# gcorso/disco-diffdock

Hardware: AMD Instinct MI355X
Metric: complexes/sec, 20-step 40-sample inference (higher is better)
Workload: dtype f32

## Files before the change

disco_diffdock_amd/csrc/ddk_capi.hip:

```cpp
#include <math.h>
#include <algorithm>
#include <cmath>
#include <string.h>

#include "model.h"
#include "k_conv_common.h"

using namespace ddk;

namespace ddk {


int fail(ddk_ctx* ctx, int code, const std::string& msg) {
  if (ctx) ctx->err = msg;
  return code;
}

int hip_fail(ddk_ctx* ctx, hipError_t e, const char* what) {
  return fail(ctx, DDK_ERR_HIP, std::string(what) + ": " + hipGetErrorString(e));
}

hipError_t ctx_malloc(ddk_ctx* ctx, void** p, size_t bytes) {
  *p = nullptr;
  if (ctx->alloc_limit > 0 && ctx->dev_bytes + (int64_t)bytes > ctx->alloc_limit) { ctx->alloc_refusals++; return hipErrorOutOfMemory; }
// ... 240 lines not shown
        }
        if (n_x > 0 && (int)xs.size() == n_x) {
          std::vector<TileDesc> keep_t; std::vector<TRow> keep_r, x_r; std::vector<int> x_off;
          for (int t = t_first; t < (int)tiles.size(); ++t) {
            if (std::find(xs.begin(), xs.end(), t) != xs.end()) { x_r.push_back(trows[t]); x_off.push_back(tiles[t].w0 >> 16); }
            else { keep_t.push_back(tiles[t]); keep_r.push_back(trows[t]); }
          }
          for (int u = 0; u < 3 * n_x; ++u) {
            keep_r[u].has_x = true; keep_r[u].xpair = u % 3;
            for (int j = 0; j < 4; ++j) keep_r[u].xr[j] = x_r[u / 3].r[j];
            keep_t[u].w0 |= 0x80 | ((u % 3) << 8) | ((x_off[u / 3] / 4) << 10);
          }
          tiles.resize(t_first); trows.resize(t_first);
          tiles.insert(tiles.end(), keep_t.begin(), keep_t.end());
          trows.insert(trows.end(), keep_r.begin(), keep_r.end());
        }
      }
      tiles.back().w0 |= (vec ? FL_V : FL_S) << 2;
    }
  }
  if (mode == 3 && !ctx->cfg.deterministic) {
    L.n_cols = 0;
    for (int t = 0; t < (int)tiles.size(); ++t) {
      const bool prev_flushes = t > 0 && ((tiles[t - 1].w0 >> 2) & 3) != FL_NONE;
      if (t == 0 || prev_flushes || t - L.col_start[L.n_cols - 1] == 2) {
        if (L.n_cols >= 16) return fail(ctx, DDK_ERR_INVALID, "too many output columns");
        if (t > 0 && !prev_flushes) tiles[t - 1].w0 |= FL_V << 2;
        L.col_start[L.n_cols++] = t;
      }
    }
  }
  L.n_tiles = (int)tiles.size();
  L.col_start[L.n_cols] = L.n_tiles;
  L.h_tiles = tiles;

  rowmap.assign((size_t)L.n_tiles * 32, -1);
  rowscale.assign((size_t)L.n_tiles * 32, 0.f);
  for (int t = 0; t < L.n_tiles; ++t) {
    const TRow& tr = trows[t];
    for (int rq = 0; rq < 4; ++rq)
      for (int hh = 0; hh < 2; ++hh)
        for (int j = 0; j < 4; ++j) {
          if (tr.has_x && rq == 3) {
            rowmap[(size_t)t * 32 + 8 * rq + 4 * hh + j] = tr.xr[j].wbase + 8 * tr.col + 2 * tr.xpair + hh;
            rowscale[(size_t)t * 32 + 8 * rq + 4 * hh + j] = tr.xr[j].scale;
            continue;
          }
          const int k = 8 * tr.col + 2 * rq + hh;
          if (!tr.ok[j] || k >= L.n_out[tr.blk[j]]) continue;
          rowmap[(size_t)t * 32 + 8 * rq + 4 * hh + j] = tr.r[j].wbase + k;
          rowscale[(size_t)t * 32 + 8 * rq + 4 * hh + j] = tr.r[j].scale;
        }
  }
  std::vector<int> cnt(L.W, 0);
  for (int r : rowmap) if (r >= 0) cnt[r]++;
  for (int r = 0; r < L.W; ++r) if (cnt[r] != 1) return fail(ctx, DDK_ERR_INVALID, "internal: weight row map is not a bijection");
  return DDK_OK;
}

static int fold_batch_norm(ddk_ctx* ctx, const std::string& pre, const int* out, float* mean, float* scale, float* bias) {
  for (int i = 0; i < XW; ++i) { mean[i] = 0.f; scale[i] = 1.f; bias[i] = 0.f; }
  const int nf = out[0] + out[1] + out[2] + out[3];
  const HostTensor* bw = find_w(ctx, pre + ".weight", {nf});
  const HostTensor* bb = find_w(ctx, pre + ".bias", {out[0]});
  const HostTensor* bm = find_w(ctx, pre + ".running_mean", {out[0]});
  const HostTensor* bv = find_w(ctx, pre + ".running_var", {nf});
  if (!bw || !bb || !bm || !bv) return DDK_ERR_INVALID;
  int ch = 0, f = 0;
  const int dims[4] = {1, 3, 3, 1};
  for (int b = 0; b < 4; ++b)
    for (int m = 0; m < out[b]; ++m, ++f) {
      const float sc = powf(bv->data[f] + 1e-5f, -0.5f) * bw->data[f];
      for (int d = 0; d < dims[b]; ++d, ++ch) {
        scale[ch] = sc;
        if (b == 0) { mean[ch] = bm->data[m]; bias[ch] = bb->data[m]; }
      }
    }
  return DDK_OK;
}

static int pack_x3(ddk_ctx* ctx, ConvLayerDev& L, int NG, const std::vector<float>& w1all, const std::vector<float>& w2all,
                   const std::vector<float>& b2all) {
  const size_t w1sz = 3 * 9 * 64 * 4, w2sz = (size_t)L.n_tiles * 9 * 64 * 4, b2sz = (size_t)L.n_tiles * 32;
  bool exact = true;
  auto split = [&exact](float v, uint16_t& hi, uint16_t& mid, uint16_t& lo) {
    const _Float16 h = (_Float16)v;
    const float r1 = v - (float)h;
    const _Float16 m = (_Float16)r1;
    const _Float16 l = (_Float16)(r1 - (float)m);
    memcpy(&hi, &h, 2); memcpy(&mid, &m, 2); memcpy(&lo, &l, 2);
    const double back = (double)(float)h + (double)(float)m + (double)(float)l;
    if (std::fabs(v) >= 0.5f ? back != (double)v : std::fabs(back - (double)v) > 0x1p-25) exact = false;
  };
  auto range_scale = [](const float* v, size_t n, const float* v2, size_t n2) {
    float m = 0.f;
    for (size_t i = 0; i < n; ++i) m = std::max(m, std::fabs(v[i]));
    for (size_t i = 0; i < n2; ++i) m = std::max(m, std::fabs(v2[i]));
    int e = 0;
    std::frexp(std::max(m, 0x1p-40f), &e);
    return std::ldexp(1.0f, 15 - e);
  };
  std::vector<uint8_t> w2x((size_t)(NG * L.n_tiles + 4) * W2X_TILE_BYTES, 0), w1x((size_t)NG * 3 * W1X_TILE_BYTES, 0);
  auto frags = [&](const float* src, float sc, uint8_t* dst) {
    for (int r = 0; r < 36; ++r)
      for (int lane = 0; lane < 64; ++lane) {
        const float v = src[((size_t)(r / 4) * 64 + lane) * 4 + (r & 3)] * sc;
        const int s_ = r / 8, i = r % 8;
        const size_t off = s_ < 4 ? (size_t)s_ * 1024 + lane * 16 + 2 * i : (size_t)4096 + lane * 8 + 2 * i;
        uint16_t h, m, l;
        split(v, h, m, l);
        memcpy(dst + off, &h, 2); memcpy(dst + W2X_LIMB_BYTES + off, &m, 2); memcpy(dst + 2 * W2X_LIMB_BYTES + off, &l, 2);
      }
  };
  for (int g = 0; g < NG; ++g) {
    const float* w2 = w2all.data() + g * w2sz;
    const float* w1 = w1all.data() + g * w1sz;
    const float* b2 = b2all.data() + g * b2sz;
    const float sc1 = range_scale(w1, w1sz, nullptr, 0), sc2 = range_scale(w2, w2sz, nullptr, 0);
    L.w1s[g] = sc1; L.w2s[g] = sc2;
    for (int t = 0; t < L.n_tiles; ++t) {
      uint8_t* rec = w2x.data() + ((size_t)g * L.n_tiles + t) * W2X_TILE_BYTES;
      frags(w2 + (size_t)t * 2304, sc2, rec);
      memcpy(rec + W2X_BIAS_OFF, b2 + (size_t)t * 32, 128);
      const int32_t dq[2] = {x_tile_word(L.h_tiles[t].w0), L.h_tiles[t].chan0};
      if (dq[0] < 0) return fail(ctx, DDK_ERR_INVALID, "internal: a vector tile of the conv layout does not sit on a T1O / T1E row quad");
      memcpy(rec + W2X_DESC_OFF, dq, 8);
    }
    for (int T = 0; T < 3; ++T) frags(w1 + (size_t)T * 2304, sc1, w1x.data() + ((size_t)g * 3 + T) * W1X_TILE_BYTES);
  }
  if (!exact) return fail(ctx, DDK_ERR_INVALID, "internal: the three-limb fp16 split of a conv weight is not exact");
  L.h_w2x = w2x; L.h_w1x = w1x;
  L.epi_ok = conv_epilogue_shapes_ok(L.h_tiles);
  L.limbs = ctx->cfg.conv_kernel == 3 ? 3 : 2;
  if (ctx->host_only) return DDK_OK;
  L.w2x = (uint8_t*)dev_alloc(ctx, w2x.size());
  L.w1x = (uint8_t*)dev_alloc(ctx, w1x.size());
  if (!L.w2x || !L.w1x) return fail(ctx, DDK_ERR_NOMEM, "device allocation failed while packing conv weights (three-limb f16)");
  if (hipMemcpy(L.w2x, w2x.data(), w2x.size(), hipMemcpyHostToDevice) != hipSuccess ||
      hipMemcpy(L.w1x, w1x.data(), w1x.size(), hipMemcpyHostToDevice) != hipSuccess)
    return fail(ctx, DDK_ERR_HIP, "three-limb weight upload failed");
  return DDK_OK;
}

static int build_conv_layer(ddk_ctx* ctx, int mode, int l, ConvLayerDev& L) {
  const ddk_config& c = ctx->cfg;
  const int ns = c.ns;
  std::vector<int> rowmap;
  std::vector<float> rowscale;
  std::vector<TileDesc> tiles;
  int rc = build_layout(ctx, mode, l, L, rowmap, rowscale, tiles);
  if (rc) return rc;
  const int NG = mode == 0 ? 4 : 9;
  L.n_groups = NG;
  const int ne = 3 * ns;
  auto fc_name = [&](int g) { return mode == 0 ? "conv_layers." + std::to_string(l) + ".fc." + std::to_string(g) : "conv_layers." + std::to_string(9 * l + g) + ".fc"; };
  const std::string lin2 = mode == 0 ? ".4" : ".3";
  if (ctx->weights.find(fc_name(0) + ".0.weight") == ctx->weights.end()) {
    L.has_weights = false;
    return DDK_OK;
  }
  L.has_weights = true;
  const size_t w1sz = 3 * 9 * 64 * 4, b1sz = 3 * 2 * 16, w2sz = (size_t)L.n_tiles * 9 * 64 * 4, b2sz = (size_t)L.n_tiles * 32;
  std::vector<float> w1all(NG * w1sz, 0.f), b1all(NG * b1sz, 0.f), w2all(NG * w2sz, 0.f), b2all(NG * b2sz, 0.f);
  for (int g = 0; g < NG; ++g) {
    const std::string f = fc_name(g);
    const HostTensor* W1 = find_w(ctx, f + ".0.weight", {ne, ne});
    const HostTensor* B1 = find_w(ctx, f + ".0.bias", {ne});
    const HostTensor* W2 = find_w(ctx, f + lin2 + ".weight", {L.W, ne});
    const HostTensor* B2 = find_w(ctx, f + lin2 + ".bias", {L.W});
    if (!W1 || !B1 || !W2 || !B2) return DDK_ERR_INVALID;
    float* w1 = w1all.data() + g * w1sz;
    float* b1 = b1all.data() + g * b1sz;
    float* w2 = w2all.data() + g * w2sz;
    float* b2 = b2all.data() + g * b2sz;
    for (int T = 0; T < 3; ++T) {
      for (int s = 0; s < 36; ++s)
        for (int lane = 0; lane < 64; ++lane) {
          const int hidden = 32 * T + (lane & 31), hh = lane >> 5;
          w1[(((size_t)T * 9 + s / 4) * 64 + lane) * 4 + (s & 3)] = hidden < ne ? W1->data[(size_t)hidden * ne + kin_of(s, hh)] : 0.f;
        }
      for (int hh = 0; hh < 2; ++hh)
        for (int r = 0; r < 16; ++r) {
          const int hidden = 32 * T + d_row(r, hh);
          b1[(T * 2 + hh) * 16 + r] = hidden < ne ? B1->data[hidden] : 0.f;
        }
    }
    for (int t = 0; t < L.n_tiles; ++t) {
      for (int s = 0; s < 36; ++s)
        for (int lane = 0; lane < 64; ++lane) {
          const int row = rowmap[(size_t)t * 32 + (lane & 31)], hh = lane >> 5;
          w2[(((size_t)t * 9 + s / 4) * 64 + lane) * 4 + (s & 3)] =
              row >= 0 ? W2->data[(size_t)row * ne + hid_of(s, hh)] * rowscale[(size_t)t * 32 + (lane & 31)] : 0.f;
        }
      for (int hh = 0; hh < 2; ++hh)
        for (int r = 0; r < 16; ++r) {
          const int row = rowmap[(size_t)t * 32 + d_row(r, hh)];
          b2[((size_t)t * 2 + hh) * 16 + r] = row >= 0 ? B2->data[row] * rowscale[(size_t)t * 32 + d_row(r, hh)] : 0.f;
        }
    }
  }
  if (mode == 0) {
    L.h_wn.assign((size_t)2 * 4 * NE * NS, 0.f);
    L.h_bnp.assign((size_t)2 * 4 * NE, 0.f);
    const int recv_g[2][2] = {{0, 1}, {2, 3}}, send_g[2][2] = {{0, 3}, {1, 2}};
    for (int type = 0; type < 2; ++type)
      for (int slot = 0; slot < 4; ++slot) {
        const int g = slot < 2 ? recv_g[type][slot] : send_g[type][slot - 2];
        const HostTensor* W1 = find_w(ctx, fc_name(g) + ".0.weight", {ne, ne});
        const HostTensor* B1 = find_w(ctx, fc_name(g) + ".0.bias", {ne});
        if (!W1 || !B1) return DDK_ERR_INVALID;
        const int col0 = slot < 2 ? NS : 2 * NS;
        for (int o = 0; o < ne; ++o) {
          const size_t row = ((size_t)(type * 4 + slot) * NE + pre_pos(o));
          for (int k = 0; k < NS; ++k) L.h_wn[row * NS + k] = W1->data[(size_t)o * ne + col0 + k];
          L.h_bnp[row] = slot < 2 ? B1->data[o] : 0.f;
        }
      }
  }
  const int n_bn = mode == 0 ? 1 : NG;
  L.h_bn_mean.assign((size_t)n_bn * XW, 0.f);
  L.h_bn_scale.assign((size_t)n_bn * XW, 1.f);
  L.h_bn_bias.assign((size_t)n_bn * XW, 0.f);
  if (c.batch_norm)
// ... 428 lines not shown
```

disco_diffdock_amd/csrc/ddk_internal.h:

```cpp
#pragma once
#include <hip/hip_runtime.h>
#include <stdint.h>

#include <map>
#include <string>
#include <vector>

#include "../../include/ddk.h"
#include "../../include/ddk_debug.h"

namespace ddk {

constexpr int NS = 24;
constexpr int NV = 6;
constexpr int XW = 2 * NS + 6 * NV;
constexpr int NE = 3 * NS;
constexpr int OFF_P = NS;
constexpr int OFF_Q = NS + 3 * NV;
constexpr int OFF_C = NS + 6 * NV;

constexpr int F_A = 0;
constexpr int F_C = NS;
constexpr int F_T1O = 2 * NS;
constexpr int F_T1E = F_T1O + 6 * NV;
constexpr int F_PQ = F_T1E + 6 * NV;
constexpr int F_STRIDE = F_PQ + 12;
static_assert(F_STRIDE == 132 && NV == 6, "F row layout");

constexpr int F_T2O = F_STRIDE;
constexpr int F_T2E = F_T2O + 24;
constexpr int F_STRIDE2 = F_T2E + 24;
static_assert(F_STRIDE2 == 180, "F row layout (l<=2)");

constexpr int CONV_WAVES = 8;
constexpr int CONV_BLOCK_EDGES = 32 * CONV_WAVES;
constexpr int W2_TILE_FLOATS = 9 * 64 * 4 + 32 + 4;
constexpr int CONV_LDS_FLOATS = CONV_WAVES * 32 * F_STRIDE + 2 * W2_TILE_FLOATS + 16;
constexpr size_t CONV_LDS_BYTES = (size_t)CONV_LDS_FLOATS * 4;
static_assert(CONV_LDS_BYTES <= 160 * 1024, "LDS budget");
template <int MODE> struct ConvTraits;
template <> struct ConvTraits<0> { static constexpr int WAVES = CONV_WAVES, FS = F_STRIDE; };
template <> struct ConvTraits<1> { static constexpr int WAVES = 6, FS = F_STRIDE2; };
template <int MODE> constexpr size_t conv_lds_bytes() { return (size_t)(ConvTraits<MODE>::WAVES * 32 * ConvTraits<MODE>::FS + 2 * W2_TILE_FLOATS + 16) * 4; }
static_assert(conv_lds_bytes<1>() <= 160 * 1024, "LDS budget (l<=2)");
constexpr int CONV_MAX_GROUPS = 9;
constexpr int W2X_LIMB_BYTES = 4 * 1024 + 512;
constexpr int W2X_BIAS_OFF = 3 * W2X_LIMB_BYTES;
constexpr int W2X_DESC_OFF = W2X_BIAS_OFF + 128;
constexpr int W2X_TILE_BYTES = W2X_DESC_OFF + 16;
constexpr int W1X_TILE_BYTES = 3 * W2X_LIMB_BYTES;
constexpr int CONV_TRACE_TILES = 1024;
constexpr int FX_A = 0, FX_C = NS, FX_R = 2 * NS, FX_PQ = FX_R + 6 * NV, FX_STRIDE = FX_PQ + 12 + 4;
static_assert(FX_STRIDE == 100 && FX_A == F_A && FX_C == F_C, "F row layout (three-limb f16)");
constexpr int W2X_STAGES = 4;
constexpr size_t CONV_X_LDS_BYTES = (size_t)CONV_WAVES * 32 * FX_STRIDE * 4 + W2X_STAGES * W2X_TILE_BYTES + 16;
static_assert(CONV_X_LDS_BYTES <= 160 * 1024 && W2X_TILE_BYTES % 16 == 0, "LDS budget (three-limb f16)");

enum TileKind : int {
  T_RA = 0,
  T_RT = 1,
  T_TV = 2,
  T_RTS = 3
};
enum FlushMode : int { FL_NONE = 0, FL_S = 1 , FL_V = 2  };

struct TileDesc {
  int32_t w0;
  int32_t chan0;
  int32_t pad0, pad1;
};
static inline TileDesc make_tile(int kind, int f_off, int flush, int nrq, int chan0) {
  TileDesc t;
  t.w0 = kind | (flush << 2) | (nrq << 4) | (f_off << 16);
  t.chan0 = chan0; t.pad0 = 0; t.pad1 = 0;
  return t;
}

constexpr int32_t X_TILE_L2 = 1 << 24;
static inline int32_t x_tile_word(int32_t w0) {
  const int kind = w0 & 3, f_off = w0 >> 16;
  int nf = f_off;
  if (kind == T_RT || kind == T_RTS) nf = FX_PQ + (f_off - F_PQ);
  else if (kind == T_TV && f_off >= F_T2O) {
    const bool odd = f_off < F_T2E;
    const int rel = f_off - (odd ? F_T2O : F_T2E), q = rel / 12;
    if (f_off >= F_STRIDE2 || rel % 12 || q > 1 || (w0 & 0xc000)) return -1;
    nf = FX_R + 12 * (odd ? q : q + 1);
    return (w0 & 0xffff) | (nf << 16) | X_TILE_L2;
  } else if (kind == T_TV) {
    const bool odd = f_off < F_T1E;
    const int rel = f_off - (odd ? F_T1O : F_T1E), q = rel / 12;
    if (f_off < F_T1O || f_off >= F_PQ || rel % 12 || (w0 & 0xc000)) return -1;
    nf = FX_R + 12 * q;
    for (int half = 0; half < 2; ++half) {
      const bool first = 4 * q + 2 * half < NV;
      if (first != odd) w0 |= 0x4000 << half;
    }
  }
  return (w0 & 0xffff) | (nf << 16);
}

struct ConvLayerDev {
  int n_tiles = 0;
  bool has_weights = false;
  int W = 0;
  int din = 0, dout = 0;
  float* w1p[4] = {};
  float* b1p[4] = {};
  float* w2r[4] = {};
  uint8_t* w1x = nullptr;
  uint8_t* w2x = nullptr;
  float w1s[CONV_MAX_GROUPS] = {1, 1, 1, 1, 1, 1, 1, 1, 1}, w2s[CONV_MAX_GROUPS] = {1, 1, 1, 1, 1, 1, 1, 1, 1};
  int limbs = 2;
  bool epi_ok = false;
  int n_cols = 0;
  int col_start[17] = {};
  float* wn = nullptr;
  float* bnp = nullptr;
  std::vector<float> h_wn, h_bnp;
  float* bn_mean = nullptr;
  float* bn_scale = nullptr;
  float* bn_bias = nullptr;
  std::vector<std::vector<float>> h_w1p, h_b1p, h_w2p, h_b2p;
  std::vector<float> h_bn_mean, h_bn_scale, h_bn_bias;
  int n_groups = 4;
  std::vector<TileDesc> h_tiles;
  std::vector<uint8_t> h_w1x, h_w2x;
  int n_in[4] = {}, n_out[4] = {}, blk_off[4] = {};
  int in_mul[4] = {}, out_mul[4] = {};
};

constexpr int PRE_W = 4 * NE;
static inline int pre_pos(int o) {
  const int r32 = o < 64 ? o % 32 : o - 64, hh = (r32 >> 2) & 1;
  return o < 64 ? hh * 36 + (o / 32) * 16 + (r32 & 3) + 4 * (r32 >> 3) : hh * 36 + 32 + (r32 & 3);
}

struct HostTensor {
  std::vector<int64_t> shape;
// ... 119 lines not shown
```

disco_diffdock_amd/csrc/k_conv_x.hip:

```cpp
#include <stdlib.h>

#include "k_conv_common.h"

#ifdef X3_TWO_LIMBS
#define conv_x3_kernel conv_x2_kernel
#define launch_conv_fused_x launch_conv_fused_x2
#define conv_prepare_device_x conv_prepare_device_x2
#include "k_conv_x_epi2_gen.inc"
#define X3_SUM(r) D0[r]
#define X3_TAIL3(a_lh, a_hm) (void)(a_lh); D0 = MFMA16(a_hm, HT.mh, D0); D0 = MFMA16(a_hm, HT.hm, D0);
#define X3_STEP(MF, ah, am, al, bh, bm, bl)   \
  (void)(al);                                 \
  D0 = MF(ah, bm, D0);                        \
  D0 = MF(am, bh, D0);                        \
  D0 = MF(ah, bh, D0);
#define X3_FRAG(f, off) f.h = *reinterpret_cast<const f16x8*>(ringl + (off)); f.m = *reinterpret_cast<const f16x8*>(ringl + W2X_LIMB_BYTES + (off));
#define X3_TAIL_LO(SO) th
#define X3_TRIO(mask) { __builtin_amdgcn_sched_group_barrier(0x008, 1, 0); __builtin_amdgcn_sched_group_barrier(mask, 1, 0); __builtin_amdgcn_sched_group_barrier(0x100, 1, 0); }
#define X3_RIDERS_0 X3_PAIR(0x100) X3_TRIO(0x020) X3_TRIO(0x020)
#define X3_RIDERS_1 X3_PAIR(0x100) X3_PAIR(0x100) X3_TRIO(0x100)
#define X3_RIDERS_2 X3_PAIR(0x100) X3_PAIR(0x100) X3_BARE
#define X3_RIDERS_3 X3_PAIR(0x100) X3_PAIR(0x100) X3_PAIR(0x100)
#define X3_TAIL_BARES X3_BARE X3_BARE
#else
#include "k_conv_x_epi_gen.inc"
#define X3_SUM(r) (D0[r] + D1[r])
#define X3_TAIL3(a_lh, a_hm) D0 = MFMA16(a_hm, HT.mh, D0); D1 = MFMA16(a_lh, HT.hl, D1); D0 = MFMA16(a_hm, HT.hm, D0);
#define X3_STEP(MF, ah, am, al, bh, bm, bl)   \
  D1 = MF(ah, bl, D1);                        \
  D0 = MF(ah, bm, D0);                        \
  D1 = MF(al, bh, D1);                        \
  D0 = MF(ah, bh, D0);                        \
  D1 = MF(am, bm, D1);                        \
  D0 = MF(am, bh, D0);
#define X3_FRAG(f, off) f.h = *reinterpret_cast<const f16x8*>(ringl + (off)); f.m = *reinterpret_cast<const f16x8*>(ringl + W2X_LIMB_BYTES + (off)); f.l = *reinterpret_cast<const f16x8*>(ringl + 2 * W2X_LIMB_BYTES + (off));
#define X3_TAIL_LO(SO) *reinterpret_cast<const f16x4*>(ringt + (SO) + 2 * W2X_LIMB_BYTES + 4096)
#define X3_RIDERS_0 X3_PAIR(0x100) X3_PAIR(0x020) X3_PAIR(0x100) X3_PAIR(0x020) X3_PAIR(0x100) X3_PAIR(0x100)
#define X3_RIDERS_1 X3_PAIR(0x100) X3_PAIR(0x100) X3_PAIR(0x100) X3_PAIR(0x100) X3_PAIR(0x100) X3_PAIR(0x100)
#define X3_RIDERS_2 X3_PAIR(0x100) X3_PAIR(0x100) X3_PAIR(0x100) X3_BARE X3_BARE X3_BARE
#define X3_RIDERS_3 X3_PAIR(0x100) X3_PAIR(0x100) X3_PAIR(0x100) X3_PAIR(0x100) X3_BARE X3_BARE
#define X3_TAIL_BARES X3_BARE X3_BARE X3_BARE
#endif

namespace ddk {

typedef _Float16 f16x8 __attribute__((ext_vector_type(8)));
typedef _Float16 f16x4 __attribute__((ext_vector_type(4)));
typedef unsigned int u32x4 __attribute__((vector_size(16)));
#define MFMA16(a, b, c) __builtin_amdgcn_mfma_f32_32x32x16_f16((a), (b), (c), 0, 0, 0)
#define MFMA8(a, b, c) __builtin_amdgcn_mfma_f32_32x32x8f16((a), (b), (c), 0, 0, 0)

__device__ __forceinline__ float range_scale(float m, float& inv) {
  const uint32_t eb = max((__float_as_uint(m) >> 23) & 0xffu, 87u);
  inv = __uint_as_float((eb - 14u) << 23);
  return __uint_as_float((268u - eb) << 23);
}

struct Limb3 { _Float16 h, m, l; };
__device__ __forceinline__ Limb3 split3(float v) {
  Limb3 q;
  q.h = (_Float16)v;
  const float r1 = v - (float)q.h;
  q.m = (_Float16)r1;
  q.l = (_Float16)(r1 - (float)q.m);
  return q;
}

struct Limbs {
  f16x8 hi[4], mid[4], lo[4];
  f16x4 thi, tmid, tlo;
};
struct TailB { f16x8 mh, hl, hm; };
__device__ __forceinline__ TailB make_tailb(const Limbs& L) {
  TailB t;
  t.mh = __builtin_shufflevector(L.tmid, L.thi, 0, 1, 2, 3, 4, 5, 6, 7);
  t.hl = __builtin_shufflevector(L.thi, L.tlo, 0, 1, 2, 3, 4, 5, 6, 7);
  t.hm = __builtin_shufflevector(L.thi, L.tmid, 0, 1, 2, 3, 4, 5, 6, 7);
  return t;
}

__device__ __forceinline__ void make_limbs(Limbs& L, const float (&v)[36], float scale) {
#pragma unroll
  for (int s = 0; s < 4; ++s)
#pragma unroll
    for (int i = 0; i < 8; ++i) { const Limb3 q = split3(v[8 * s + i] * scale); L.hi[s][i] = q.h; L.mid[s][i] = q.m; L.lo[s][i] = q.l; }
#pragma unroll
  for (int i = 0; i < 4; ++i) { const Limb3 q = split3(v[32 + i] * scale); L.thi[i] = q.h; L.tmid[i] = q.m; L.tlo[i] = q.l; }
}

__device__ __forceinline__ void lds_barrier() {
  __builtin_amdgcn_fence(__ATOMIC_RELEASE, "workgroup", "local");
  __builtin_amdgcn_s_barrier();
  __builtin_amdgcn_fence(__ATOMIC_ACQUIRE, "workgroup", "local");
}

struct Frag16 { f16x8 h, m, l; };
__device__ __forceinline__ Frag16 lds_frag16(const char* stage, int s, int lane) {
  Frag16 f;
  f.h = *reinterpret_cast<const f16x8*>(stage + s * 1024 + lane * 16);
  f.m = *reinterpret_cast<const f16x8*>(stage + W2X_LIMB_BYTES + s * 1024 + lane * 16);
  f.l = *reinterpret_cast<const f16x8*>(stage + 2 * W2X_LIMB_BYTES + s * 1024 + lane * 16);
  return f;
}

struct SegF { float m1, m2, m4, m8, m16; bool tail, valid; };
__device__ __forceinline__ SegF make_segf(const SegCtl& c) {
  SegF f;
  f.m1 = c.m1 ? 1.0f : 0.0f; f.m2 = c.m2 ? 1.0f : 0.0f; f.m4 = c.m4 ? 1.0f : 0.0f; f.m8 = c.m8 ? 1.0f : 0.0f; f.m16 = c.m16 ? 1.0f : 0.0f;
  f.tail = c.tail; f.valid = c.valid;
  return f;
}
#define SEGF_STEP(CTRL, m)                                                                                                  \
  _Pragma("unroll") for (int i = 0; i < N; ++i) {                                                                           \
    if (N >= 3) asm volatile("v_fmac_f32_dpp %0, %0, %1 " CTRL " bound_ctrl:1" : "+v"(xv[i]) : "v"(m));                     \
    else asm volatile("s_nop 1\n\tv_fmac_f32_dpp %0, %0, %1 " CTRL " bound_ctrl:1" : "+v"(xv[i]) : "v"(m));                 \
  }
template <bool DET, int N>
__device__ __forceinline__ void segf_add_n(float* dst, int stride, float (&xv)[N], const SegF& c) {
#pragma unroll
  for (int i = 0; i < N; ++i) xv[i] = c.valid ? xv[i] : 0.0f;
  asm volatile("s_nop 1" ::: "memory");
  SEGF_STEP("row_shr:1 row_mask:0xf bank_mask:0xf", c.m1)
  SEGF_STEP("row_shr:2 row_mask:0xf bank_mask:0xf", c.m2)
  SEGF_STEP("row_shr:4 row_mask:0xf bank_mask:0xf", c.m4)
  SEGF_STEP("row_shr:8 row_mask:0xf bank_mask:0xf", c.m8)
  SEGF_STEP("row_bcast:15 row_mask:0xa bank_mask:0xf", c.m16)
  if (c.tail) {
#pragma unroll
    for (int i = 0; i < N; ++i) {
      if (DET) dst[i * stride] = xv[i];
      else unsafeAtomicAdd(dst + i * stride, xv[i]);
    }
  }
}
// ... 9 lines not shown
    a01[0] = fmaf(f0.x, d0, fmaf(f0.y, d1, a01[0]));
    a01[1] = fmaf(f1.x, d0, fmaf(f1.y, d1, a01[1]));
    a01[2] = fmaf(f2.x, d0, fmaf(f2.y, d1, a01[2]));
    float (&a23)[3] = X23 ? accX[rq] : accV[rq];
    a23[0] = fmaf(f0.z, d2, fmaf(f0.w, d3, a23[0]));
    a23[1] = fmaf(f1.z, d2, fmaf(f1.w, d3, a23[1]));
    a23[2] = fmaf(f2.z, d2, fmaf(f2.w, d3, a23[2]));
  }
}
__device__ __forceinline__ void tv_rows_l2(const f32x16& D, f32x4 f0, f32x4 f1, f32x4 f2, float (&accY)[3][3]) {
#pragma unroll
  for (int rq = 0; rq < TVQ; ++rq) {
    const float d0 = D[4 * rq], d1 = D[4 * rq + 1], d2 = D[4 * rq + 2], d3 = D[4 * rq + 3];
    accY[rq][0] = fmaf(f0.x, d0, fmaf(f0.y, d1, fmaf(f0.z, d2, fmaf(f0.w, d3, accY[rq][0]))));
    accY[rq][1] = fmaf(f1.x, d0, fmaf(f1.y, d1, fmaf(f1.z, d2, fmaf(f1.w, d3, accY[rq][1]))));
    accY[rq][2] = fmaf(f2.x, d0, fmaf(f2.y, d1, fmaf(f2.z, d2, fmaf(f2.w, d3, accY[rq][2]))));
  }
}
template <int MODE>
__device__ __forceinline__ void tile_epilogue_s(int w0, const f32x16& D, const float* Fp, f32x4 f0, float (&accA)[4], float (&accV)[4][3],
                                                float (&accX)[4][3], float (&accY)[3][3]) {
  const int kind = w0 & 3;
  if (MODE == 1 && kind == T_TV && (w0 & X_TILE_L2)) {
    const f32x4 f1 = ldv4(Fp + 4), f2 = ldv4(Fp + 8);
    tv_rows_l2(D, f0, f1, f2, accY);
  } else if (kind == T_TV) {
    const f32x4 f1 = ldv4(Fp + 4), f2 = ldv4(Fp + 8);
    switch ((w0 >> 14) & 3) {
      case 0: tv_rows<false, false>(D, f0, f1, f2, accV, accX); break;
      case 1: tv_rows<true, false>(D, f0, f1, f2, accV, accX); break;
      case 2: tv_rows<false, true>(D, f0, f1, f2, accV, accX); break;
      default: tv_rows<true, true>(D, f0, f1, f2, accV, accX); break;
    }
  } else if (kind == T_RA) {
#pragma unroll
    for (int rq = 0; rq < 4; ++rq)
      accA[rq] = fmaf(f0.x, D[4 * rq], fmaf(f0.y, D[4 * rq + 1], fmaf(f0.z, D[4 * rq + 2], fmaf(f0.w, D[4 * rq + 3], accA[rq]))));
  } else if (kind == T_RT) {
#pragma unroll
    for (int rq = 0; rq < 4; ++rq)
      accV[rq][0] = fmaf(f0.x, D[4 * rq], fmaf(f0.y, D[4 * rq + 1], fmaf(f0.z, D[4 * rq + 2], fmaf(f0.w, D[4 * rq + 3], accV[rq][0]))));
  } else {
#pragma unroll
    for (int rq = 0; rq < 4; ++rq) accV[rq][0] = fmaf(f0.x, D[4 * rq], fmaf(f0.y, D[4 * rq + 1], accV[rq][0]));
  }
}

constexpr float UNIT_PROLOGUE_TILES = 6.5f;
template <bool GATHER, bool SPLIT, bool DET, bool TRACE = false, int MODE = 0>
__global__ __launch_bounds__(64 * CONV_WAVES) void conv_x3_kernel(ConvXArgs AX) {
  static_assert(!SPLIT || GATHER, "the GEMM1 split exists for the gather path");
  static_assert(MODE == 0 || (!SPLIT && !DET && !TRACE), "the confidence model runs the plain paths");
  int trace_n = 0;
  auto stamp = [&](int phase) {
    if constexpr (TRACE) {
      if (AX.trace_coarse == 1 && phase < 4) return;
      if (blockIdx.x == 0 && (threadIdx.x & 63) == 0 && trace_n < CONV_TRACE_TILES)
        AX.trace[((threadIdx.x >> 6) * CONV_TRACE_TILES + trace_n) * 8 + phase] = (uint32_t)__builtin_amdgcn_s_memtime();
      if (phase == 3) ++trace_n;
    }
  };
  bool first_tile = true;
  auto stamp_epi = [&](int slot) {
    if constexpr (TRACE) {
      if (AX.trace_coarse != 2 || first_tile) return;
      if (blockIdx.x == 0 && (threadIdx.x & 63) == 0 && trace_n < CONV_TRACE_TILES)
        AX.trace[((threadIdx.x >> 6) * CONV_TRACE_TILES + trace_n) * 8 + slot] = (uint32_t)__builtin_amdgcn_s_memtime();
    }
  };
  auto stamp_unit = [&](int slot, int value) {
    if constexpr (TRACE) {
      if (AX.trace_coarse != 1) return;
      if (blockIdx.x == 0 && (threadIdx.x & 63) == 0 && trace_n < CONV_TRACE_TILES)
        AX.trace[((threadIdx.x >> 6) * CONV_TRACE_TILES + trace_n) * 8 + slot] = slot == 1 ? (uint32_t)value : (uint32_t)__builtin_amdgcn_s_memtime();
      if (slot == 2) ++trace_n;
    }
  };
  const ConvKArgs& A = AX.k;
  constexpr int WAVES = CONV_WAVES, FS = FX_STRIDE, BLOCK_EDGES = 32 * WAVES;
  extern __shared__ __attribute__((aligned(16))) float lds[];
  const int tid = threadIdx.x, lane = tid & 63, wave = tid >> 6;
  float* F = lds + wave * (32 * FS);
  char* ring = reinterpret_cast<char*>(lds + WAVES * (32 * FS));
  int* blk_slot = reinterpret_cast<int*>(ring + W2X_STAGES * W2X_TILE_BYTES);
  const int el = lane & 31;
  const int hh = lane >> 5;
  const bool g2_shared = A.sum_g2 != nullptr;
  int gb_v = 0, ge_v = 0;
  if (lane < A.n_active) {
    gb_v = A.gbeg[lane];
    ge_v = A.gend[lane];
  }
  const int nb_v = (ge_v - gb_v + BLOCK_EDGES - 1) / BLOCK_EDGES;
  int pend_v = nb_v;
#pragma unroll
  for (int d = 1; d < 16; d *= 2) {
    const int t = __shfl_up(pend_v, d, 64);
    if (lane >= d) pend_v += t;
  }
  const int pbeg_v = pend_v - nb_v;
  int bs4 = __builtin_amdgcn_readlane(pend_v, 15);
  if constexpr (DET) {
    if (A.det_nr > 0) bs4 = A.det_rng[A.det_nr];
  }
  float* Fr = F + el * FS;
  const float inv_s3 = 0.57735026918962576451f, inv_s2 = 0.70710678118654752440f;
  const int n_tiles = A.n_tiles;
  constexpr int REC16 = W2X_TILE_BYTES / 16;
  const int grp = wave >> 2;
  const uint32_t fo0 = 16u * tid, fo1 = 16u * min(tid + 64 * WAVES, REC16 - 1);
  constexpr bool ASM_EPI = GATHER && SPLIT && !DET && MODE == 0;
  const unsigned ring0_u = (unsigned)(WAVES * 32 * FS * 4), ringb_u = ring0_u + 64u * hh, ringw0_u = ring0_u + fo0, ringw1_u = ring0_u + fo1;
  const unsigned fra_u = (unsigned)((wave * 32 + el) * FS * 4), hh4_u = 4u * hh, hh12_u = 12u * hh;
  int t0_, t1_, t2_, sel_, pk0_, pk1_, pk2_;
  unsigned long long sv_;
  (void)ringb_u; (void)ringw0_u; (void)ringw1_u; (void)fra_u; (void)hh4_u; (void)hh12_u;

  const int nwg = gridDim.x;
  const int full = bs4 >= nwg ? (bs4 / nwg) * nwg : 0;
  const int rest = bs4 - full;
  int split = 1;
  if (rest > 0) {
    float best = 1e30f;
    for (int sp = 1; sp <= A.n_cols; ++sp) {
      const float cost = (float)((rest * sp + nwg - 1) / nwg) * ((float)n_tiles / (float)sp + UNIT_PROLOGUE_TILES);
      if (cost < best - 1e-6f) { best = cost; split = sp; }
    }
  }
  const int n_units = full + rest * split;

  int unit = blockIdx.x;
  for (;;) {
    if (unit >= n_units) break;
    stamp(4);
    first_tile = true;
    int unit_next = 0;
    if (tid == 0) unit_next = nwg + atomicAdd(A.counter, 1);
    int blk = unit, t_begin = 0, t_end = n_tiles;
    if (unit >= full) {
      const int r = unit - full, c = r % split;
      blk = full + r / split;
      t_begin = A.col_start[(c * A.n_cols) / split];
      t_end = A.col_start[((c + 1) * A.n_cols) / split];
    }
    int g = __popcll(__ballot(lane < 16 && blk >= pend_v));
    int gbeg = __builtin_amdgcn_readlane(gb_v, g), gend = __builtin_amdgcn_readlane(ge_v, g);
    int bstart = __builtin_amdgcn_readlane(pbeg_v, g);
    if constexpr (DET) {
      if (A.det_nr > 0) {
        const DetRange R_ = det_find(A.det_rng, A.det_nr, blk);
        g = R_.g; gbeg = R_.beg; gend = R_.end; bstart = R_.bstart;
      }
    }
    const int e0 = gbeg + BLOCK_EDGES * (blk - bstart) + 32 * wave;
    const int nvalid = min(32, gend - e0);
    const bool valid = el < nvalid;
    const int e = nvalid > 0 ? e0 + min(el, nvalid - 1) : gend - 1;
    const int sn = A.src[e], dn = A.dst[e];

    const int gw = (int)((A.wmap >> (4 * g)) & 15);
    const char* wrec = reinterpret_cast<const char*>(A.w2x) + (size_t)gw * n_tiles * W2X_TILE_BYTES;
    {
      const char* wr0 = wrec + (size_t)t_begin * W2X_TILE_BYTES;
      const char* wr1 = wrec + (size_t)min(t_begin + 1, t_end - 1) * W2X_TILE_BYTES;
      const char* wr2 = wrec + (size_t)min(t_begin + 2, t_end - 1) * W2X_TILE_BYTES;
      const float4 r0 = *reinterpret_cast<const float4*>(wr0 + fo0), r1 = *reinterpret_cast<const float4*>(wr0 + fo1);
      const float4 r2 = *reinterpret_cast<const float4*>(wr1 + fo0), r3 = *reinterpret_cast<const float4*>(wr1 + fo1);
      const float4 r4 = *reinterpret_cast<const float4*>(wr2 + fo0), r5 = *reinterpret_cast<const float4*>(wr2 + fo1);
      *reinterpret_cast<float4*>(ring + fo0) = r0;
      *reinterpret_cast<float4*>(ring + fo1) = r1;
      *reinterpret_cast<float4*>(ring + W2X_TILE_BYTES + fo0) = r2;
      *reinterpret_cast<float4*>(ring + W2X_TILE_BYTES + fo1) = r3;
      *reinterpret_cast<float4*>(ring + 2 * W2X_TILE_BYTES + fo0) = r4;
      *reinterpret_cast<float4*>(ring + 2 * W2X_TILE_BYTES + fo1) = r5;
    }

    const SegF seg = make_segf(make_segctl(sn, el, nvalid, valid));
    stamp(5);

    const float4 shv = ld4(A.sh + (size_t)e * 4);
    float4 mainv[NS / 4];
    float2 pv2[3 * NV / 2];
    {
      const float* xr = A.x + (size_t)dn * XW;
#pragma unroll
      for (int j = 0; j < NS / 4; ++j) mainv[j] = ld4(xr + (hh ? OFF_C : 0) + 4 * j);
#pragma unroll
      for (int j = 0; j < 3 * NV / 2; ++j) pv2[j] = ld2(xr + (hh ? OFF_Q : OFF_P) + 2 * j);
    }

    Limbs H;
    TailB HT;
    float osc, bsc2;
    {
      float h[36];
      const char* w1 = reinterpret_cast<const char*>(A.w1x) + (size_t)gw * 3 * W1X_TILE_BYTES;
      if constexpr (SPLIT) {
        float4 psv[9], pdv[9];
        {
          const float* ps = A.pre + ((size_t)sn * 4 + (gw & 1)) * NE + 36 * hh;
          const float* pd = A.pre + ((size_t)dn * 4 + 2 + (gw >> 1)) * NE + 36 * hh;
#pragma unroll
          for (int j = 0; j < 9; ++j) { psv[j] = ld4(ps + 4 * j); pdv[j] = ld4(pd + 4 * j); }
        }
        float bin[12];
        {
          const float* pe = A.edge_attr + (size_t)e * NS + 12 * hh;
#pragma unroll
          for (int j = 0; j < 3; ++j) {
            const float4 a = ld4(pe + 4 * j);
            bin[4 * j + 0] = a.x; bin[4 * j + 1] = a.y; bin[4 * j + 2] = a.z; bin[4 * j + 3] = a.w;
          }
        }
        float m1 = 0.0f;
#pragma unroll
        for (int j = 0; j < 12; ++j) m1 = fmaxf(m1, fabsf(bin[j]));
        m1 = fmaxf(m1, __shfl_xor(m1, 32));
        float inv1;
        const float s1 = range_scale(m1, inv1);
        f16x8 b0h, b0m, b0l;
        f16x4 b1h, b1m, b1l;
#pragma unroll
        for (int i = 0; i < 8; ++i) { const Limb3 q = split3(bin[i] * s1); b0h[i] = q.h; b0m[i] = q.m; b0l[i] = q.l; }
#pragma unroll
        for (int i = 0; i < 4; ++i) { const Limb3 q = split3(bin[8 + i] * s1); b1h[i] = q.h; b1m[i] = q.m; b1l[i] = q.l; }
        const f16x8 b1_mh = __builtin_shufflevector(b1m, b1h, 0, 1, 2, 3, 4, 5, 6, 7), b1_hl = __builtin_shufflevector(b1h, b1l, 0, 1, 2, 3, 4, 5, 6, 7),
                    b1_hm = __builtin_shufflevector(b1h, b1m, 0, 1, 2, 3, 4, 5, 6, 7);
        const float bsc = s1 * A.w1s[gw], usc = inv1 * A.w1u[gw];
#pragma unroll
        for (int T = 0; T < 3; ++T) {
          f32x16 D0, D1;
#pragma unroll
          for (int j = 0; j < 4; ++j) {
            if (T < 2 || j == 0) {
              const float4 u = psv[4 * T + j], w = pdv[4 * T + j];
              D0[4 * j + 0] = (u.x + w.x) * bsc; D0[4 * j + 1] = (u.y + w.y) * bsc; D0[4 * j + 2] = (u.z + w.z) * bsc; D0[4 * j + 3] = (u.w + w.w) * bsc;
            } else {
              D0[4 * j + 0] = 0.0f; D0[4 * j + 1] = 0.0f; D0[4 * j + 2] = 0.0f; D0[4 * j + 3] = 0.0f;
            }
          }
#pragma unroll
          for (int r = 0; r < 16; ++r) D1[r] = 0.0f;
          const char* wt = w1 + (size_t)T * W1X_TILE_BYTES;
          {
            const f16x8 ah = *reinterpret_cast<const f16x8*>(wt + lane * 16);
            const f16x8 am = *reinterpret_cast<const f16x8*>(wt + W2X_LIMB_BYTES + lane * 16);
            const f16x8 al = *reinterpret_cast<const f16x8*>(wt + 2 * W2X_LIMB_BYTES + lane * 16);
            X3_STEP(MFMA16, ah, am, al, b0h, b0m, b0l)
          }
          {
            const f16x4 ah = *reinterpret_cast<const f16x4*>(wt + 1024 + lane * 16);
            const f16x4 am = *reinterpret_cast<const f16x4*>(wt + W2X_LIMB_BYTES + 1024 + lane * 16);
            const f16x4 al = *reinterpret_cast<const f16x4*>(wt + 2 * W2X_LIMB_BYTES + 1024 + lane * 16);
            const f16x8 a_hm = __builtin_shufflevector(ah, am, 0, 1, 2, 3, 4, 5, 6, 7), a_lh = __builtin_shufflevector(al, ah, 0, 1, 2, 3, 4, 5, 6, 7);
            D0 = MFMA16(a_hm, b1_mh, D0);
#ifndef X3_TWO_LIMBS
            D1 = MFMA16(a_lh, b1_hl, D1);
#else
            (void)a_lh; (void)b1_hl;
#endif
            D0 = MFMA16(a_hm, b1_hm, D0);
          }
          const int nr = T < 2 ? 16 : 4;
#pragma unroll
          for (int r = 0; r < 16; ++r)
            if (r < nr) h[16 * T + r] = fmaxf(X3_SUM(r), 0.0f) * usc;
        }
      } else {
        float bin[36];
        {
          const float *pe, *pxs, *pxd;
          if (GATHER) {
            pe = A.edge_attr + (size_t)e * NS + 12 * hh;
            pxs = A.x + (size_t)sn * XW + 12 * hh;
            pxd = A.x + (size_t)dn * XW + 12 * hh;
          } else {
            pe = A.edge_attr + (size_t)e * NE + 12 * hh;
            pxs = pe + NS;
            pxd = pe + 2 * NS;
          }
#pragma unroll
          for (int j = 0; j < 3; ++j) {
            const float4 a = ld4(pe + 4 * j), b = ld4(pxs + 4 * j), c = ld4(pxd + 4 * j);
            bin[4 * j + 0] = a.x; bin[4 * j + 1] = a.y; bin[4 * j + 2] = a.z; bin[4 * j + 3] = a.w;
            bin[12 + 4 * j + 0] = b.x; bin[12 + 4 * j + 1] = b.y; bin[12 + 4 * j + 2] = b.z; bin[12 + 4 * j + 3] = b.w;
            bin[24 + 4 * j + 0] = c.x; bin[24 + 4 * j + 1] = c.y; bin[24 + 4 * j + 2] = c.z; bin[24 + 4 * j + 3] = c.w;
          }
        }
        float m1 = 0.0f;
#pragma unroll
        for (int j = 0; j < 36; ++j) m1 = fmaxf(m1, fabsf(bin[j]));
        m1 = fmaxf(m1, __shfl_xor(m1, 32));
        float inv1;
        const float s1 = range_scale(m1, inv1);
        Limbs Bn;
        make_limbs(Bn, bin, s1);
        const float bsc = s1 * A.w1s[gw], usc = inv1 * A.w1u[gw];
        const float* b1 = A.b1p + (size_t)gw * (3 * 2 * 16);
#pragma unroll
        for (int T = 0; T < 3; ++T) {
          f32x16 D0, D1;
          const float* bp = b1 + (T * 2 + hh) * 16;
#pragma unroll
          for (int j = 0; j < 4; ++j) {
            const float4 b = ld4(bp + 4 * j);
            D0[4 * j + 0] = b.x * bsc; D0[4 * j + 1] = b.y * bsc; D0[4 * j + 2] = b.z * bsc; D0[4 * j + 3] = b.w * bsc;
          }
#pragma unroll
          for (int r = 0; r < 16; ++r) D1[r] = 0.0f;
          const char* wt = w1 + (size_t)T * W1X_TILE_BYTES;
#pragma unroll
          for (int s = 0; s < 4; ++s) {
            const f16x8 ah = *reinterpret_cast<const f16x8*>(wt + s * 1024 + lane * 16);
            const f16x8 am = *reinterpret_cast<const f16x8*>(wt + W2X_LIMB_BYTES + s * 1024 + lane * 16);
            const f16x8 al = *reinterpret_cast<const f16x8*>(wt + 2 * W2X_LIMB_BYTES + s * 1024 + lane * 16);
            X3_STEP(MFMA16, ah, am, al, Bn.hi[s], Bn.mid[s], Bn.lo[s])
          }
          {
            const f16x4 ah = *reinterpret_cast<const f16x4*>(wt + 4096 + lane * 8);
            const f16x4 am = *reinterpret_cast<const f16x4*>(wt + W2X_LIMB_BYTES + 4096 + lane * 8);
            const f16x4 al = *reinterpret_cast<const f16x4*>(wt + 2 * W2X_LIMB_BYTES + 4096 + lane * 8);
            X3_STEP(MFMA8, ah, am, al, Bn.thi, Bn.tmid, Bn.tlo)
          }
          const int nr = T < 2 ? 16 : 4;
#pragma unroll
          for (int r = 0; r < 16; ++r)
            if (r < nr) h[16 * T + r] = fmaxf(X3_SUM(r), 0.0f) * usc;
        }
      }
      float m2 = 0.0f;
#pragma unroll
      for (int j = 0; j < 36; ++j) m2 = fmaxf(m2, h[j]);
      m2 = fmaxf(m2, __shfl_xor(m2, 32));
      float inv2;
      const float s2 = range_scale(m2, inv2);
      stamp(6);
      make_limbs(H, h, s2);
      HT = make_tailb(H);
      bsc2 = s2 * A.w2s[gw];
      osc = inv2 * A.w2u[gw];
    }

    const float s0 = shv.x, vx = shv.y, vy = shv.z, vz = shv.w;
    {
      const int o_main_dst = hh ? FX_C : FX_A, r0 = hh ? NV : 0;
#pragma unroll
      for (int j = 0; j < NS / 4; ++j) *reinterpret_cast<float4*>(Fr + o_main_dst + 4 * j) = mainv[j];
      float pv[3 * NV];
#pragma unroll
      for (int j = 0; j < 3 * NV / 2; ++j) { pv[2 * j] = pv2[j].x; pv[2 * j + 1] = pv2[j].y; }
#pragma unroll
      for (int m = 0; m < NV; ++m) {
        const float px = pv[3 * m], py = pv[3 * m + 1], pz = pv[3 * m + 2];
        Fr[FX_PQ + (m < 4 ? 4 * hh + m : 8 + 2 * hh + (m - 4))] = (px * vx + py * vy + pz * vz) * inv_s3;
        const int r = r0 + m;
        float* Pr = Fr + FX_R + 12 * (r >> 2) + (r & 3);
        Pr[0] = px;
        Pr[4] = py;
        Pr[8] = pz;
      }
    }
    stamp(7);
    lds_barrier();

    float* node_row = (g2_shared && g == 2) ? A.sum_g2 + (size_t)(sn - A.g2_node_off) * XW
                                            : A.sum + ((size_t)sn * A.n_slots + ((A.slots >> (2 * g)) & 3)) * XW;
    if constexpr (DET) {
      if (nvalid > 0) {
        const int sn0 = __shfl(sn, 0, 32), snl = __shfl(sn, nvalid - 1, 32);
        const bool first_cont = e0 > gbeg && A.src[e0 - 1] == sn0;
        const bool last_cont = e0 + nvalid < gend && A.src[e0 + nvalid] == snl;
        float* prow = A.part + ((size_t)(blk * WAVES + wave) * 2) * XW;
        if (sn == sn0 && first_cont) node_row = prow;
        else if (sn == snl && last_cont) node_row = prow + XW;
      }
    }
    const bool shared2_ = g2_shared && g == 2;
    const float* sumbase = shared2_ ? A.sum_g2 : A.sum;
    const unsigned vrow = shared2_ ? (unsigned)(sn - A.g2_node_off) * (unsigned)(XW * 4)
                                   : ((unsigned)sn * (unsigned)A.n_slots + ((A.slots >> (2 * g)) & 3u)) * (unsigned)(XW * 4);
    const unsigned long long tail_mask = __ballot(seg.tail);
    const float oscv = seg.valid ? osc : 0.0f;
    (void)sumbase; (void)vrow; (void)tail_mask; (void)oscv;
    float accA[4], accV[4][3], accX[4][3];
    float accY[3][3];
#pragma unroll
    for (int rq = 0; rq < 4; ++rq) {
      accA[rq] = 0.0f; accV[rq][0] = 0.0f; accV[rq][1] = 0.0f; accV[rq][2] = 0.0f; accX[rq][0] = 0.0f; accX[rq][1] = 0.0f; accX[rq][2] = 0.0f;
      if (rq < 3) { accY[rq][0] = 0.0f; accY[rq][1] = 0.0f; accY[rq][2] = 0.0f; }
    }
    const char* ringl = ring + lane * 16;
    const char* ringt = ring + lane * 8;
    const char* ringb = ring + hh * 64;
    char* ringw0 = ring + fo0;
    char* ringw1 = ring + fo1;
    const __amdgpu_buffer_rsrc_t rsrc = __builtin_amdgcn_make_buffer_rsrc(const_cast<char*>(wrec), 0, 0x7fffffff, 0x00020000);
    int rec_soff = (t_begin + 3) * W2X_TILE_BYTES;
    Frag16 p0;
    p0.h = *reinterpret_cast<const f16x8*>(ringl); p0.m = *reinterpret_cast<const f16x8*>(ringl + W2X_LIMB_BYTES);
#ifndef X3_TWO_LIMBS
    p0.l = *reinterpret_cast<const f16x8*>(ringl + 2 * W2X_LIMB_BYTES);
#endif
    int w0, chan0;
    {
      const int2 dq = *reinterpret_cast<const int2*>(ring + W2X_DESC_OFF);
      w0 = __builtin_amdgcn_readfirstlane(dq.x); chan0 = __builtin_amdgcn_readfirstlane(dq.y);
    }
    const bool grp_s = __builtin_amdgcn_readfirstlane(grp) != 0;
    auto finish_tile = [&](int w0x, int chan0x, const f32x16& D, f32x4 f0x) {
      if (w0x & 0x80) {
        const f32x4 g0 = ldv4(Fr + ((w0x >> 8) & 0x3c));
        const float xv = fmaf(g0.x, D[12], fmaf(g0.y, D[13], fmaf(g0.z, D[14], g0.w * D[15])));
        const int xp = (w0x >> 8) & 3;
        if (xp == 0) accA[0] += xv; else if (xp == 1) accA[1] += xv; else accA[2] += xv;
      }
      const int fl = (w0x >> 2) & 3;
      if (fl) {
        const int nrq = (w0x >> 4) & 7;
        if (fl == FL_S && nrq == 4) {
          float m4[4];
#pragma unroll
          for (int rq = 0; rq < 4; ++rq) m4[rq] = osc * fmaf(accA[rq], s0, accV[rq][0]);
          segf_add_n<DET, 4>(node_row + chan0x + hh, 2, m4, seg);
        }
#pragma unroll
        for (int rq = 0; rq < 4; ++rq) {
          if (rq < nrq && !(fl == FL_S && nrq == 4)) {
            if (fl == FL_S) {
              float m1v[1] = {osc * fmaf(accA[rq], s0, accV[rq][0])};
              segf_add_n<DET, 1>(node_row + chan0x + 2 * rq + hh, 1, m1v, seg);
            } else {
              float* d = node_row + chan0x + 3 * (2 * rq + hh);
              const float sa = accA[rq], wx = vx * inv_s2, wy = vy * inv_s2, wz = vz * inv_s2;
              const float X0 = accX[rq][0], X1 = accX[rq][1], X2 = accX[rq][2];
              float m3[3] = {osc * fmaf(X1, wz, fmaf(-X2, wy, fmaf(sa, vx, s0 * accV[rq][0]))),
                             osc * fmaf(X2, wx, fmaf(-X0, wz, fmaf(sa, vy, s0 * accV[rq][1]))),
                             osc * fmaf(X0, wy, fmaf(-X1, wx, fmaf(sa, vz, s0 * accV[rq][2])))};
              if constexpr (MODE == 1) {
                const float Y0 = accY[rq < 3 ? rq : 0][0], Y1 = accY[rq < 3 ? rq : 0][1], Y2 = accY[rq < 3 ? rq : 0][2];
                const float dv = (Y0 * vx + Y1 * vy + Y2 * vz) * (1.0f / 3.0f), n3 = (vx * vx + vy * vy + vz * vz) * (1.0f / 9.0f);
                m3[0] += osc * (dv * vx - Y0 * n3); m3[1] += osc * (dv * vy - Y1 * n3); m3[2] += osc * (dv * vz - Y2 * n3);
              }
              segf_add_n<DET, 3>(d, 1, m3, seg);
            }
          }
          accA[rq] = 0.0f; accV[rq][0] = 0.0f; accV[rq][1] = 0.0f; accV[rq][2] = 0.0f; accX[rq][0] = 0.0f; accX[rq][1] = 0.0f; accX[rq][2] = 0.0f;
          if (MODE == 1 && rq < 3) { accY[rq][0] = 0.0f; accY[rq][1] = 0.0f; accY[rq][2] = 0.0f; }
        }
        if ((w0x & 3) == T_RTS) {
#pragma unroll
          for (int rq = 0; rq < 4; ++rq) accV[rq][0] = fmaf(f0x.z, D[4 * rq + 2], f0x.w * D[4 * rq + 3]);
        }
      }
    };
#define X3_PAIR(mask) { __builtin_amdgcn_sched_group_barrier(0x008, 1, 0); __builtin_amdgcn_sched_group_barrier(mask, 1, 0); }
#define X3_BARE { __builtin_amdgcn_sched_group_barrier(0x008, 1, 0); }
#define X3_BURST_BODY(ST)                                                                                                                    \
      Frag16 p1; X3_FRAG(p1, SO + 1024)                                                                                                      \
      const f32x4 f0 = ldv4(Fp);                                                                                                             \
                                    \
      const u32x4 st0 = __builtin_amdgcn_raw_buffer_load_b128(rsrc, (int)fo0, rec_soff, 0);                                                  \
      const u32x4 st1 = __builtin_amdgcn_raw_buffer_load_b128(rsrc, (int)fo1, rec_soff, 0);                                                  \
      rec_soff += W2X_TILE_BYTES;                                                                                                            \
      X3_STEP(MFMA16, p0.h, p0.m, p0.l, H.hi[0], H.mid[0], H.lo[0])                                                                         \
      X3_RIDERS_0                                                                                                                            \
      __builtin_amdgcn_sched_barrier(0);                                                                                                     \
      Frag16 q2; X3_FRAG(q2, SO + 2048)                                                                                                      \
      const f16x4 th = *reinterpret_cast<const f16x4*>(ringt + SO + 4096);                                                                   \
      const f16x4 tm = *reinterpret_cast<const f16x4*>(ringt + SO + W2X_LIMB_BYTES + 4096);                                                  \
      const f16x4 tl = X3_TAIL_LO(SO);                                                                                                       \
      X3_STEP(MFMA16, p1.h, p1.m, p1.l, H.hi[1], H.mid[1], H.lo[1])                                                                         \
      X3_RIDERS_1                                                                                                                            \
      __builtin_amdgcn_sched_barrier(0);                                                                                                     \
      Frag16 q3; X3_FRAG(q3, SO + 3072)                                                                                                      \
      X3_STEP(MFMA16, q2.h, q2.m, q2.l, H.hi[2], H.mid[2], H.lo[2])                                                                         \
      X3_RIDERS_2                                                                                                                            \
      __builtin_amdgcn_sched_barrier(0);                                                                                                     \
      const int2 dq = *reinterpret_cast<const int2*>(ring + SN + W2X_DESC_OFF);                                                              \
      X3_FRAG(p0, SN)           \
      X3_STEP(MFMA16, q3.h, q3.m, q3.l, H.hi[3], H.mid[3], H.lo[3])                                                                         \
      X3_RIDERS_3                                                                                                                            \
      __builtin_amdgcn_sched_barrier(0);
#define X3_TILE(ST)                                                                                                                          \
    {                                                                                                                                        \
      constexpr int SO = (ST) * W2X_TILE_BYTES, SN = (((ST) + 1) & 3) * W2X_TILE_BYTES, SW = (((ST) + 3) & 3) * W2X_TILE_BYTES;              \
                      \
      __builtin_amdgcn_s_setprio(1);                                                                                                         \
      stamp(0);                                                                                                                              \
                                                        \
      const float* Fp = Fr + ((w0 >> 16) & 0xff);                                                                                            \
      f32x16 D0, D1;                                                                                                                         \
      _Pragma("unroll") for (int r = 0; r < 16; ++r) { D0[r] = 0.0f; D1[r] = 0.0f; }                                                         \
      __builtin_amdgcn_sched_barrier(0);                                                                                                     \
      X3_BURST_BODY(ST)                                                                                                                      \
      {                          \
        const f16x8 a_hm = __builtin_shufflevector(th, tm, 0, 1, 2, 3, 4, 5, 6, 7), a_lh = __builtin_shufflevector(tl, th, 0, 1, 2, 3, 4, 5, 6, 7); \
        X3_TAIL3(a_lh, a_hm)                                                                                                                 \
      }                                                                                                                                      \
      X3_TAIL_BARES                                                                                                                          \
      __builtin_amdgcn_sched_barrier(0);                                                                                                     \
      __builtin_amdgcn_s_setprio(0);                                                                                                         \
      stamp(1);                                                                                                                              \
      if (grp_s) lds_barrier();                                    \
      stamp(2);                                                                                                                              \
                                                                            \
      if constexpr (ASM_EPI) {                                                                                                               \
        const unsigned fpa_u = fra_u + 4u * (unsigned)((w0 >> 16) & 0xff);                                                                   \
        const int chan4_ = chan0 * 4;                                                                                                        \
        X3_EPI_##ST();                                                                                                                       \
      } else {                                                                                                                               \
      const float4 bs0 = ld4(reinterpret_cast<const float*>(ringb + SO + W2X_BIAS_OFF)), bs1 = ld4(reinterpret_cast<const float*>(ringb + SO + W2X_BIAS_OFF + 16)); \
      const float4 bs2 = ld4(reinterpret_cast<const float*>(ringb + SO + W2X_BIAS_OFF + 32)), bs3 = ld4(reinterpret_cast<const float*>(ringb + SO + W2X_BIAS_OFF + 48)); \
      *reinterpret_cast<u32x4*>(ringw0 + SW) = st0;                                                                                          \
      *reinterpret_cast<u32x4*>(ringw1 + SW) = st1;                                                                                          \
                                                                                             \
      D0[0] = fmaf(bs0.x, bsc2, X3_SUM(0)); D0[1] = fmaf(bs0.y, bsc2, X3_SUM(1)); D0[2] = fmaf(bs0.z, bsc2, X3_SUM(2)); D0[3] = fmaf(bs0.w, bsc2, X3_SUM(3)); \
      D0[4] = fmaf(bs1.x, bsc2, X3_SUM(4)); D0[5] = fmaf(bs1.y, bsc2, X3_SUM(5)); D0[6] = fmaf(bs1.z, bsc2, X3_SUM(6)); D0[7] = fmaf(bs1.w, bsc2, X3_SUM(7)); \
      D0[8] = fmaf(bs2.x, bsc2, X3_SUM(8)); D0[9] = fmaf(bs2.y, bsc2, X3_SUM(9)); D0[10] = fmaf(bs2.z, bsc2, X3_SUM(10)); D0[11] = fmaf(bs2.w, bsc2, X3_SUM(11)); \
      D0[12] = fmaf(bs3.x, bsc2, X3_SUM(12)); D0[13] = fmaf(bs3.y, bsc2, X3_SUM(13)); D0[14] = fmaf(bs3.z, bsc2, X3_SUM(14)); D0[15] = fmaf(bs3.w, bsc2, X3_SUM(15)); \
      if ((w0 & 0x8e) == 0) {                                      \
        if (w0 & 1) {                                                                                                                        \
          _Pragma("unroll") for (int rq = 0; rq < 4; ++rq)                                                                                   \
            accV[rq][0] = fmaf(f0.x, D0[4 * rq], fmaf(f0.y, D0[4 * rq + 1], fmaf(f0.z, D0[4 * rq + 2], fmaf(f0.w, D0[4 * rq + 3], accV[rq][0])))); \
        } else {                                                                                                                             \
          _Pragma("unroll") for (int rq = 0; rq < 4; ++rq)                                                                                   \
            accA[rq] = fmaf(f0.x, D0[4 * rq], fmaf(f0.y, D0[4 * rq + 1], fmaf(f0.z, D0[4 * rq + 2], fmaf(f0.w, D0[4 * rq + 3], accA[rq])))); \
        }                                                                                                                                    \
      } else {                                                                                                                               \
        tile_epilogue_s<MODE>(w0, D0, Fp, f0, accA, accV, accX, accY);                                                                       \
        finish_tile(w0, chan0, D0, f0);                                                                                                      \
      }                                                                                                                                      \
      }                                                                                                                                      \
      w0 = __builtin_amdgcn_readfirstlane(dq.x); chan0 = __builtin_amdgcn_readfirstlane(dq.y);                                               \
      stamp_epi(7);                                                                                                                          \
      stamp(3);                                                                                                                              \
      first_tile = false;                                                                                                                    \
      if (!grp_s) lds_barrier();                                                               \
    }
    for (int t = t_begin;;) {
      X3_TILE(0)
      if (++t >= t_end) break;
      X3_TILE(1)
      if (++t >= t_end) break;
      X3_TILE(2)
      if (++t >= t_end) break;
      X3_TILE(3)
      if (++t >= t_end) break;
    }
#undef X3_PAIR
#undef X3_BARE
#undef X3_TILE
#undef X3_BURST_BODY
    stamp_unit(0, 0);
    stamp_unit(1, t_end - t_begin);
    if (tid == 0) *blk_slot = unit_next;
    lds_barrier();
    unit = __builtin_amdgcn_readfirstlane(*blk_slot);
    stamp_unit(2, 0);
  }
}

#ifndef X3_TWO_LIMBS
__global__ void split3_probe_kernel(const float* x, int64_t n, int group, float* hi, float* mid, float* lo, float* scale) {
  const int64_t i = (int64_t)blockIdx.x * blockDim.x + threadIdx.x;
  if (i >= n) return;
  const int64_t g0 = (i / group) * group;
  float m = 0.0f;
  for (int64_t k = g0; k < g0 + group && k < n; ++k) m = fmaxf(m, fabsf(x[k]));
  float inv;
  const float s = range_scale(m, inv);
  const Limb3 q = split3(x[i] * s);
  hi[i] = (float)q.h; mid[i] = (float)q.m; lo[i] = (float)q.l; scale[i] = s;
}

hipError_t launch_split3_probe(const float* x, int64_t n, int group, float* hi, float* mid, float* lo, float* scale, hipStream_t s) {
  if (n <= 0) return hipSuccess;
  hipLaunchKernelGGL(split3_probe_kernel, dim3((unsigned)((n + 255) / 256)), dim3(256), 0, s, x, n, group, hi, mid, lo, scale);
  return hipGetLastError();
}

#endif

template <bool GATHER, bool SPLIT, bool DET>
static hipError_t launch_x_t(const ConvXArgs& k, int n_cu, hipStream_t s) {
  hipLaunchKernelGGL((conv_x3_kernel<GATHER, SPLIT, DET>), dim3(n_cu), dim3(64 * CONV_WAVES), CONV_X_LDS_BYTES, s, k);
  return hipGetLastError();
}

template <bool GATHER, bool SPLIT, bool DET>
static hipError_t attr_x_t() {
  return hipFuncSetAttribute(reinterpret_cast<const void*>(&conv_x3_kernel<GATHER, SPLIT, DET>), hipFuncAttributeMaxDynamicSharedMemorySize,
                             (int)CONV_X_LDS_BYTES);
}

#ifndef X3_TWO_LIMBS
bool conv_epilogue_shapes_ok(const std::vector<TileDesc>& tiles) {
  if (tiles.empty()) return false;
  for (const TileDesc& t : tiles) {
    const int w0 = x_tile_word(t.w0);
    if (w0 < 0 || (w0 & X_TILE_L2)) return false;
    const int fl = (w0 >> 2) & 3, nrq = (w0 >> 4) & 7, kind = w0 & 3;
    if (fl == FL_S && nrq != 4) return false;
    if (fl == FL_V && nrq != 3) return false;
    if (kind == T_RTS && fl != FL_S) return false;
  }
  const int last = x_tile_word(tiles.back().w0);
  return ((last >> 2) & 3) != 0;
}
#endif

hipError_t conv_prepare_device_x() {
  hipError_t e = attr_x_t<true, true, false>();
  if (e == hipSuccess) e = attr_x_t<true, false, false>();
  if (e == hipSuccess) e = attr_x_t<false, false, false>();
  if (e == hipSuccess) e = attr_x_t<true, true, true>();
  if (e == hipSuccess) e = attr_x_t<false, false, true>();
  if (e == hipSuccess)
    e = hipFuncSetAttribute(reinterpret_cast<const void*>(&conv_x3_kernel<true, true, false, true>), hipFuncAttributeMaxDynamicSharedMemorySize,
                            (int)CONV_X_LDS_BYTES);
  if (e == hipSuccess)
    e = hipFuncSetAttribute(reinterpret_cast<const void*>(&conv_x3_kernel<true, false, false, false, 1>), hipFuncAttributeMaxDynamicSharedMemorySize,
                            (int)CONV_X_LDS_BYTES);
  if (e == hipSuccess)
    e = hipFuncSetAttribute(reinterpret_cast<const void*>(&conv_x3_kernel<false, false, false, false, 1>), hipFuncAttributeMaxDynamicSharedMemorySize,
                            (int)CONV_X_LDS_BYTES);
  return e;
}

void conv_det_fix(const ConvKArgs& k, const ConvLaunch& a, int dout, hipStream_t s);

hipError_t launch_conv_fused_x(const ConvLayerDev& L, const ConvLaunch& a, int n_cu, hipStream_t s) {
  if (a.mode != 0 && a.mode != 1) return hipErrorInvalidValue;
  ConvXArgs X;
  ConvKArgs& k = X.k;
  k.x = a.x; k.src = a.src; k.dst = a.dst; k.edge_attr = a.edge_attr; k.sh = a.sh; k.sum = a.sum;
  k.counter = a.counter;
  k.w1p = nullptr; k.b1p = L.b1p[0]; k.w2r = nullptr; k.w1x = L.w1x; k.w2x = L.w2x; k.n_tiles = L.n_tiles;
  for (int g = 0; g < CONV_MAX_GROUPS; ++g) { k.w1s[g] = L.w1s[g]; k.w1u[g] = 1.0f / L.w1s[g]; k.w2s[g] = L.w2s[g]; k.w2u[g] = 1.0f / L.w2s[g]; }
  k.n_cols = L.n_cols;
  for (int c = 0; c <= L.n_cols; ++c) k.col_start[c] = L.col_start[c];
  k.sum_g2 = a.sum_g2; k.g2_node_off = a.g2_node_off;
  k.n_groups = a.n_groups; k.n_active = a.n_active; k.n_slots = a.n_slots; k.slots = a.slots; k.wmap = a.wmap;
  if (a.gbeg) { k.gbeg = a.gbeg; k.gend = a.gend; }
  else { k.gbeg = a.tile_info + 5; k.gend = a.tile_info + 6; }
  k.pre = a.pre; k.part = a.part; k.det_rng = a.det_rng; k.det_nr = a.det_nr;
  X.trace = nullptr; X.trace_coarse = a.trace_coarse;
  if (a.mode == 1) {
    if (a.pre != nullptr || a.part != nullptr || a.trace != nullptr) return hipErrorInvalidValue;
    if (a.gather) hipLaunchKernelGGL((conv_x3_kernel<true, false, false, false, 1>), dim3(n_cu), dim3(64 * CONV_WAVES), CONV_X_LDS_BYTES, s, X);
    else hipLaunchKernelGGL((conv_x3_kernel<false, false, false, false, 1>), dim3(n_cu), dim3(64 * CONV_WAVES), CONV_X_LDS_BYTES, s, X);
    return hipGetLastError();
  }
  if (a.part != nullptr) {
    hipError_t e = (a.gather && a.pre != nullptr) ? launch_x_t<true, true, true>(X, n_cu, s)
                                                  : (!a.gather ? launch_x_t<false, false, true>(X, n_cu, s) : hipErrorInvalidValue);
    if (e != hipSuccess) return e;
    conv_det_fix(k, a, L.dout, s);
    return hipGetLastError();
  }
  if (a.gather && a.pre != nullptr && !L.epi_ok) return hipErrorInvalidValue;
  X.trace = a.trace;
  if (a.trace != nullptr) {
    if (!(a.gather && a.pre != nullptr)) return hipErrorInvalidValue;
    hipLaunchKernelGGL((conv_x3_kernel<true, true, false, true>), dim3(n_cu), dim3(64 * CONV_WAVES), CONV_X_LDS_BYTES, s, X);
    return hipGetLastError();
  }
  if (a.gather && a.pre != nullptr) return launch_x_t<true, true, false>(X, n_cu, s);
  return a.gather ? launch_x_t<true, false, false>(X, n_cu, s) : launch_x_t<false, false, false>(X, n_cu, s);
}

}
```

disco_diffdock_amd/csrc/k_conv_x_epi2_gen.inc:

```

#define X3_EPI_0() \
  asm volatile( \
    "ds_read_b128 v[0:3], %[ringb] offset:13824\n\t" \
    "ds_read_b128 v[4:7], %[ringb] offset:13840\n\t" \
    "ds_read_b128 v[8:11], %[ringb] offset:13856\n\t" \
    "ds_read_b128 v[12:15], %[ringb] offset:13872\n\t" \
    "s_waitcnt vmcnt(1)\n\t" \
    "ds_write_b128 %[rw0], %[st0] offset:41904\n\t" \
    "s_waitcnt vmcnt(0)\n\t" \
    "ds_write_b128 %[rw1], %[st1] offset:41904\n\t" \
    "s_waitcnt lgkmcnt(2)\n\t" \
    "v_fmac_f32 v16, v0, %[bsc2]\n\t" \
    "v_fmac_f32 v17, v1, %[bsc2]\n\t" \
    "v_fmac_f32 v18, v2, %[bsc2]\n\t" \
    "v_fmac_f32 v19, v3, %[bsc2]\n\t" \
    "v_fmac_f32 v20, v4, %[bsc2]\n\t" \
    "v_fmac_f32 v21, v5, %[bsc2]\n\t" \
    "v_fmac_f32 v22, v6, %[bsc2]\n\t" \
    "v_fmac_f32 v23, v7, %[bsc2]\n\t" \
    "v_fmac_f32 v24, v8, %[bsc2]\n\t" \
    "v_fmac_f32 v25, v9, %[bsc2]\n\t" \
    "v_fmac_f32 v26, v10, %[bsc2]\n\t" \
    "v_fmac_f32 v27, v11, %[bsc2]\n\t" \
    "v_fmac_f32 v28, v12, %[bsc2]\n\t" \
    "v_fmac_f32 v29, v13, %[bsc2]\n\t" \
    "v_fmac_f32 v30, v14, %[bsc2]\n\t" \
    "v_fmac_f32 v31, v15, %[bsc2]\n\t" \
    "s_and_b32 %[t0], %[w0], 3\n\t" \
    "s_bfe_u32 %[t1], %[w0], 0x2000e\n\t" \
    "s_add_i32 %[t1], %[t1], 3\n\t" \
    "s_add_i32 %[t2], %[t0], 1\n\t" \
    "s_cmp_eq_u32 %[t0], 2\n\t" \
    "s_cselect_b32 %[t2], %[t1], %[t2]\n\t" \
    "s_cmp_eq_u32 %[t0], 3\n\t" \
    "s_cselect_b32 %[sel], 7, %[t2]\n\t" \
    "s_cmp_lg_u32 %[sel], 1\n\t" \
    "s_cbranch_scc1 .Lkrare_%=\n\t" \
    "v_fmac_f32 %[aA0], v51, v19\n\t" \
    "v_fmac_f32 %[aA1], v51, v23\n\t" \
    "v_fmac_f32 %[aA2], v51, v27\n\t" \
    "v_fmac_f32 %[aA3], v51, v31\n\t" \
    "v_fmac_f32 %[aA0], v50, v18\n\t" \
    "v_fmac_f32 %[aA1], v50, v22\n\t" \
    "v_fmac_f32 %[aA2], v50, v26\n\t" \
    "v_fmac_f32 %[aA3], v50, v30\n\t" \
    "v_fmac_f32 %[aA0], v49, v17\n\t" \
    "v_fmac_f32 %[aA1], v49, v21\n\t" \
    "v_fmac_f32 %[aA2], v49, v25\n\t" \
    "v_fmac_f32 %[aA3], v49, v29\n\t" \
    "v_fmac_f32 %[aA0], v48, v16\n\t" \
    "v_fmac_f32 %[aA1], v48, v20\n\t" \
    "v_fmac_f32 %[aA2], v48, v24\n\t" \
    "v_fmac_f32 %[aA3], v48, v28\n\t" \
    ".Lkjoin_%=:\n\t" \
    "s_bitcmp0_b32 %[w0], 7\n\t" \
    "s_cbranch_scc1 .Lnp_%=\n\t" \
    "s_lshr_b32 %[t0], %[w0], 6\n\t" \
    "s_and_b32 %[t0], %[t0], 0xf0\n\t" \
    "v_add_u32 v52, %[t0], %[fra]\n\t" \
    "ds_read_b128 v[8:11], v52\n\t" \
    "s_bfe_u32 %[t1], %[w0], 0x20008\n\t" \
    "s_cmp_eq_u32 %[t1], 0\n\t" \
    "s_cselect_b32 %[pk0], 1.0, 0\n\t" \
    "s_cmp_eq_u32 %[t1], 1\n\t" \
    "s_cselect_b32 %[pk1], 1.0, 0\n\t" \
    "s_cmp_eq_u32 %[t1], 2\n\t" \
    "s_cselect_b32 %[pk2], 1.0, 0\n\t" \
    "s_waitcnt lgkmcnt(0)\n\t" \
    "v_mul_f32 v52, v11, v31\n\t" \
    "v_fmac_f32 v52, v10, v30\n\t" \
    "v_fmac_f32 v52, v9, v29\n\t" \
    "v_fmac_f32 v52, v8, v28\n\t" \
    "v_fmac_f32 %[aA0], %[pk0], v52\n\t" \
    "v_fmac_f32 %[aA1], %[pk1], v52\n\t" \
    "v_fmac_f32 %[aA2], %[pk2], v52\n\t" \
    ".Lnp_%=:\n\t" \
    "s_bfe_u32 %[t0], %[w0], 0x20002\n\t" \
    "s_cmp_eq_u32 %[t0], 0\n\t" \
    "s_cbranch_scc1 .Lnf_%=\n\t" \
    "s_cmp_eq_u32 %[t0], 2\n\t" \
    "s_cbranch_scc1 .Lfv_%=\n\t" \
    "s_cmp_eq_u32 %[sel], 7\n\t" \
    "s_cbranch_scc1 .Lfr_%=\n\t" \
    "v_fma_f32 v0, %[aA0], %[s0], %[aV00]\n\t" \
    "v_fma_f32 v1, %[aA1], %[s0], %[aV10]\n\t" \
    "v_fma_f32 v2, %[aA2], %[s0], %[aV20]\n\t" \
    "v_fma_f32 v3, %[aA3], %[s0], %[aV30]\n\t" \
    "v_mul_f32 v0, %[oscv], v0\n\t" \
    "v_mul_f32 v1, %[oscv], v1\n\t" \
    "v_mul_f32 v2, %[oscv], v2\n\t" \
    "v_mul_f32 v3, %[oscv], v3\n\t" \
    "v_mov_b32 %[aA0], 0\n\t" \
    "v_mov_b32 %[aV00], 0\n\t" \
    "v_mov_b32 %[aA1], 0\n\t" \
// ... 320 lines not shown
    "ds_read_b128 v[0:3], %[fpa] offset:16\n\t" \
    "ds_read_b128 v[4:7], %[fpa] offset:32\n\t" \
    "v_fmac_f32 %[aV00], v49, v17\n\t" \
    "v_fmac_f32 %[aV10], v49, v21\n\t" \
    "v_fmac_f32 %[aV20], v49, v25\n\t" \
    "v_fmac_f32 %[aV00], v48, v16\n\t" \
    "v_fmac_f32 %[aV10], v48, v20\n\t" \
    "v_fmac_f32 %[aV20], v48, v24\n\t" \
    "v_fmac_f32 %[aX00], v51, v19\n\t" \
    "v_fmac_f32 %[aX10], v51, v23\n\t" \
    "v_fmac_f32 %[aX20], v51, v27\n\t" \
    "v_fmac_f32 %[aX00], v50, v18\n\t" \
    "v_fmac_f32 %[aX10], v50, v22\n\t" \
    "v_fmac_f32 %[aX20], v50, v26\n\t" \
    "s_waitcnt lgkmcnt(1)\n\t" \
    "v_fmac_f32 %[aV01], v1, v17\n\t" \
    "v_fmac_f32 %[aV11], v1, v21\n\t" \
    "v_fmac_f32 %[aV21], v1, v25\n\t" \
    "v_fmac_f32 %[aV01], v0, v16\n\t" \
    "v_fmac_f32 %[aV11], v0, v20\n\t" \
    "v_fmac_f32 %[aV21], v0, v24\n\t" \
    "v_fmac_f32 %[aX01], v3, v19\n\t" \
    "v_fmac_f32 %[aX11], v3, v23\n\t" \
    "v_fmac_f32 %[aX21], v3, v27\n\t" \
    "v_fmac_f32 %[aX01], v2, v18\n\t" \
    "v_fmac_f32 %[aX11], v2, v22\n\t" \
    "v_fmac_f32 %[aX21], v2, v26\n\t" \
    "s_waitcnt lgkmcnt(0)\n\t" \
    "v_fmac_f32 %[aV02], v5, v17\n\t" \
    "v_fmac_f32 %[aV12], v5, v21\n\t" \
    "v_fmac_f32 %[aV22], v5, v25\n\t" \
    "v_fmac_f32 %[aV02], v4, v16\n\t" \
    "v_fmac_f32 %[aV12], v4, v20\n\t" \
    "v_fmac_f32 %[aV22], v4, v24\n\t" \
    "v_fmac_f32 %[aX02], v7, v19\n\t" \
    "v_fmac_f32 %[aX12], v7, v23\n\t" \
    "v_fmac_f32 %[aX22], v7, v27\n\t" \
    "v_fmac_f32 %[aX02], v6, v18\n\t" \
    "v_fmac_f32 %[aX12], v6, v22\n\t" \
    "v_fmac_f32 %[aX22], v6, v26\n\t" \
    "s_branch .Lkjoin_%=\n\t" \
    ".Lkv4_%=:\n\t" \
    "ds_read_b128 v[0:3], %[fpa] offset:16\n\t" \
    "ds_read_b128 v[4:7], %[fpa] offset:32\n\t" \
    "v_fmac_f32 %[aX00], v49, v17\n\t" \
    "v_fmac_f32 %[aX10], v49, v21\n\t" \
    "v_fmac_f32 %[aX20], v49, v25\n\t" \
    "v_fmac_f32 %[aX00], v48, v16\n\t" \
    "v_fmac_f32 %[aX10], v48, v20\n\t" \
    "v_fmac_f32 %[aX20], v48, v24\n\t" \
    "v_fmac_f32 %[aX00], v51, v19\n\t" \
    "v_fmac_f32 %[aX10], v51, v23\n\t" \
    "v_fmac_f32 %[aX20], v51, v27\n\t" \
    "v_fmac_f32 %[aX00], v50, v18\n\t" \
    "v_fmac_f32 %[aX10], v50, v22\n\t" \
    "v_fmac_f32 %[aX20], v50, v26\n\t" \
    "s_waitcnt lgkmcnt(1)\n\t" \
    "v_fmac_f32 %[aX01], v1, v17\n\t" \
    "v_fmac_f32 %[aX11], v1, v21\n\t" \
    "v_fmac_f32 %[aX21], v1, v25\n\t" \
    "v_fmac_f32 %[aX01], v0, v16\n\t" \
    "v_fmac_f32 %[aX11], v0, v20\n\t" \
    "v_fmac_f32 %[aX21], v0, v24\n\t" \
    "v_fmac_f32 %[aX01], v3, v19\n\t" \
    "v_fmac_f32 %[aX11], v3, v23\n\t" \
    "v_fmac_f32 %[aX21], v3, v27\n\t" \
    "v_fmac_f32 %[aX01], v2, v18\n\t" \
    "v_fmac_f32 %[aX11], v2, v22\n\t" \
    "v_fmac_f32 %[aX21], v2, v26\n\t" \
    "s_waitcnt lgkmcnt(0)\n\t" \
    "v_fmac_f32 %[aX02], v5, v17\n\t" \
    "v_fmac_f32 %[aX12], v5, v21\n\t" \
    "v_fmac_f32 %[aX22], v5, v25\n\t" \
    "v_fmac_f32 %[aX02], v4, v16\n\t" \
    "v_fmac_f32 %[aX12], v4, v20\n\t" \
    "v_fmac_f32 %[aX22], v4, v24\n\t" \
    "v_fmac_f32 %[aX02], v7, v19\n\t" \
    "v_fmac_f32 %[aX12], v7, v23\n\t" \
    "v_fmac_f32 %[aX22], v7, v27\n\t" \
    "v_fmac_f32 %[aX02], v6, v18\n\t" \
    "v_fmac_f32 %[aX12], v6, v22\n\t" \
    "v_fmac_f32 %[aX22], v6, v26\n\t" \
    "s_branch .Lkjoin_%=\n\t" \
    ".Lexit_%=:\n\t" \
    : [D0] "+{v[16:31]}"(D0), [aA0] "+v"(accA[0]), [aA1] "+v"(accA[1]), [aA2] "+v"(accA[2]), [aA3] "+v"(accA[3]), [aV00] "+v"(accV[0][0]), [aX00] "+v"(accX[0][0]), [aV01] "+v"(accV[0][1]), [aX01] "+v"(accX[0][1]), [aV02] "+v"(accV[0][2]), [aX02] "+v"(accX[0][2]), [aV10] "+v"(accV[1][0]), [aX10] "+v"(accX[1][0]), [aV11] "+v"(accV[1][1]), [aX11] "+v"(accX[1][1]), [aV12] "+v"(accV[1][2]), [aX12] "+v"(accX[1][2]), [aV20] "+v"(accV[2][0]), [aX20] "+v"(accX[2][0]), [aV21] "+v"(accV[2][1]), [aX21] "+v"(accX[2][1]), [aV22] "+v"(accV[2][2]), [aX22] "+v"(accX[2][2]), [aV30] "+v"(accV[3][0]), [aX30] "+v"(accX[3][0]), [aV31] "+v"(accV[3][1]), [aX31] "+v"(accX[3][1]), [aV32] "+v"(accV[3][2]), [aX32] "+v"(accX[3][2]), [t0] "=&s"(t0_), [t1] "=&s"(t1_), [t2] "=&s"(t2_), [sel] "=&s"(sel_), [pk0] "=&s"(pk0_), [pk1] "=&s"(pk1_), [pk2] "=&s"(pk2_), [sv] "=&s"(sv_) \
    : [f0] "{v[48:51]}"(f0), [st0] "v"(st0), [st1] "v"(st1), [ringb] "v"(ringb_u), [rw0] "v"(ringw0_u), [rw1] "v"(ringw1_u), [fpa] "v"(fpa_u), [fra] "v"(fra_u), [bsc2] "v"(bsc2), [oscv] "v"(oscv), [s0] "v"(s0), [vx] "v"(vx), [vy] "v"(vy), [vz] "v"(vz), [sm1] "v"(seg.m1), [sm2] "v"(seg.m2), [sm4] "v"(seg.m4), [sm8] "v"(seg.m8), [sm16] "v"(seg.m16), [vrow] "v"(vrow), [hh4] "v"(hh4_u), [hh12] "v"(hh12_u), [w0] "s"(w0), [chan4] "s"(chan4_), [tail] "s"(tail_mask), [sumbase] "s"(sumbase) \
    : "v0", "v1", "v2", "v3", "v4", "v5", "v6", "v7", "v8", "v9", "v10", "v11", "v12", "v13", "v14", "v15", "v52", "v53", "memory", "scc")

#define X3_EPI_1() \
  asm volatile( \
    "ds_read_b128 v[0:3], %[ringb] offset:27792\n\t" \
    "ds_read_b128 v[4:7], %[ringb] offset:27808\n\t" \
    "ds_read_b128 v[8:11], %[ringb] offset:27824\n\t" \
    "ds_read_b128 v[12:15], %[ringb] offset:27840\n\t" \
    "s_waitcnt vmcnt(1)\n\t" \
    "ds_write_b128 %[rw0], %[st0] offset:0\n\t" \
    "s_waitcnt vmcnt(0)\n\t" \
    "ds_write_b128 %[rw1], %[st1] offset:0\n\t" \
    "s_waitcnt lgkmcnt(2)\n\t" \
    "v_fmac_f32 v16, v0, %[bsc2]\n\t" \
    "v_fmac_f32 v17, v1, %[bsc2]\n\t" \
    "v_fmac_f32 v18, v2, %[bsc2]\n\t" \
    "v_fmac_f32 v19, v3, %[bsc2]\n\t" \
    "v_fmac_f32 v20, v4, %[bsc2]\n\t" \
    "v_fmac_f32 v21, v5, %[bsc2]\n\t" \
    "v_fmac_f32 v22, v6, %[bsc2]\n\t" \
    "v_fmac_f32 v23, v7, %[bsc2]\n\t" \
    "v_fmac_f32 v24, v8, %[bsc2]\n\t" \
    "v_fmac_f32 v25, v9, %[bsc2]\n\t" \
    "v_fmac_f32 v26, v10, %[bsc2]\n\t" \
    "v_fmac_f32 v27, v11, %[bsc2]\n\t" \
    "v_fmac_f32 v28, v12, %[bsc2]\n\t" \
    "v_fmac_f32 v29, v13, %[bsc2]\n\t" \
    "v_fmac_f32 v30, v14, %[bsc2]\n\t" \
    "v_fmac_f32 v31, v15, %[bsc2]\n\t" \
    "s_and_b32 %[t0], %[w0], 3\n\t" \
    "s_bfe_u32 %[t1], %[w0], 0x2000e\n\t" \
    "s_add_i32 %[t1], %[t1], 3\n\t" \
    "s_add_i32 %[t2], %[t0], 1\n\t" \
    "s_cmp_eq_u32 %[t0], 2\n\t" \
    "s_cselect_b32 %[t2], %[t1], %[t2]\n\t" \
    "s_cmp_eq_u32 %[t0], 3\n\t" \
    "s_cselect_b32 %[sel], 7, %[t2]\n\t" \
    "s_cmp_lg_u32 %[sel], 1\n\t" \
    "s_cbranch_scc1 .Lkrare_%=\n\t" \
    "v_fmac_f32 %[aA0], v51, v19\n\t" \
    "v_fmac_f32 %[aA1], v51, v23\n\t" \
    "v_fmac_f32 %[aA2], v51, v27\n\t" \
    "v_fmac_f32 %[aA3], v51, v31\n\t" \
    "v_fmac_f32 %[aA0], v50, v18\n\t" \
    "v_fmac_f32 %[aA1], v50, v22\n\t" \
    "v_fmac_f32 %[aA2], v50, v26\n\t" \
    "v_fmac_f32 %[aA3], v50, v30\n\t" \
    "v_fmac_f32 %[aA0], v49, v17\n\t" \
    "v_fmac_f32 %[aA1], v49, v21\n\t" \
    "v_fmac_f32 %[aA2], v49, v25\n\t" \
    "v_fmac_f32 %[aA3], v49, v29\n\t" \
    "v_fmac_f32 %[aA0], v48, v16\n\t" \
    "v_fmac_f32 %[aA1], v48, v20\n\t" \
    "v_fmac_f32 %[aA2], v48, v24\n\t" \
    "v_fmac_f32 %[aA3], v48, v28\n\t" \
    ".Lkjoin_%=:\n\t" \
    "s_bitcmp0_b32 %[w0], 7\n\t" \
    "s_cbranch_scc1 .Lnp_%=\n\t" \
    "s_lshr_b32 %[t0], %[w0], 6\n\t" \
    "s_and_b32 %[t0], %[t0], 0xf0\n\t" \
    "v_add_u32 v52, %[t0], %[fra]\n\t" \
    "ds_read_b128 v[8:11], v52\n\t" \
    "s_bfe_u32 %[t1], %[w0], 0x20008\n\t" \
    "s_cmp_eq_u32 %[t1], 0\n\t" \
    "s_cselect_b32 %[pk0], 1.0, 0\n\t" \
    "s_cmp_eq_u32 %[t1], 1\n\t" \
    "s_cselect_b32 %[pk1], 1.0, 0\n\t" \
    "s_cmp_eq_u32 %[t1], 2\n\t" \
    "s_cselect_b32 %[pk2], 1.0, 0\n\t" \
    "s_waitcnt lgkmcnt(0)\n\t" \
    "v_mul_f32 v52, v11, v31\n\t" \
    "v_fmac_f32 v52, v10, v30\n\t" \
    "v_fmac_f32 v52, v9, v29\n\t" \
    "v_fmac_f32 v52, v8, v28\n\t" \
    "v_fmac_f32 %[aA0], %[pk0], v52\n\t" \
    "v_fmac_f32 %[aA1], %[pk1], v52\n\t" \
    "v_fmac_f32 %[aA2], %[pk2], v52\n\t" \
    ".Lnp_%=:\n\t" \
    "s_bfe_u32 %[t0], %[w0], 0x20002\n\t" \
    "s_cmp_eq_u32 %[t0], 0\n\t" \
    "s_cbranch_scc1 .Lnf_%=\n\t" \
    "s_cmp_eq_u32 %[t0], 2\n\t" \
    "s_cbranch_scc1 .Lfv_%=\n\t" \
    "s_cmp_eq_u32 %[sel], 7\n\t" \
    "s_cbranch_scc1 .Lfr_%=\n\t" \
    "v_fma_f32 v0, %[aA0], %[s0], %[aV00]\n\t" \
    "v_fma_f32 v1, %[aA1], %[s0], %[aV10]\n\t" \
    "v_fma_f32 v2, %[aA2], %[s0], %[aV20]\n\t" \
    "v_fma_f32 v3, %[aA3], %[s0], %[aV30]\n\t" \
    "v_mul_f32 v0, %[oscv], v0\n\t" \
    "v_mul_f32 v1, %[oscv], v1\n\t" \
    "v_mul_f32 v2, %[oscv], v2\n\t" \
    "v_mul_f32 v3, %[oscv], v3\n\t" \
    "v_mov_b32 %[aA0], 0\n\t" \
    "v_mov_b32 %[aV00], 0\n\t" \
    "v_mov_b32 %[aA1], 0\n\t" \
// ... 320 lines not shown
    "ds_read_b128 v[0:3], %[fpa] offset:16\n\t" \
    "ds_read_b128 v[4:7], %[fpa] offset:32\n\t" \
    "v_fmac_f32 %[aV00], v49, v17\n\t" \
    "v_fmac_f32 %[aV10], v49, v21\n\t" \
    "v_fmac_f32 %[aV20], v49, v25\n\t" \
    "v_fmac_f32 %[aV00], v48, v16\n\t" \
    "v_fmac_f32 %[aV10], v48, v20\n\t" \
    "v_fmac_f32 %[aV20], v48, v24\n\t" \
    "v_fmac_f32 %[aX00], v51, v19\n\t" \
    "v_fmac_f32 %[aX10], v51, v23\n\t" \
    "v_fmac_f32 %[aX20], v51, v27\n\t" \
    "v_fmac_f32 %[aX00], v50, v18\n\t" \
    "v_fmac_f32 %[aX10], v50, v22\n\t" \
    "v_fmac_f32 %[aX20], v50, v26\n\t" \
    "s_waitcnt lgkmcnt(1)\n\t" \
    "v_fmac_f32 %[aV01], v1, v17\n\t" \
    "v_fmac_f32 %[aV11], v1, v21\n\t" \
    "v_fmac_f32 %[aV21], v1, v25\n\t" \
    "v_fmac_f32 %[aV01], v0, v16\n\t" \
    "v_fmac_f32 %[aV11], v0, v20\n\t" \
    "v_fmac_f32 %[aV21], v0, v24\n\t" \
    "v_fmac_f32 %[aX01], v3, v19\n\t" \
    "v_fmac_f32 %[aX11], v3, v23\n\t" \
    "v_fmac_f32 %[aX21], v3, v27\n\t" \
    "v_fmac_f32 %[aX01], v2, v18\n\t" \
    "v_fmac_f32 %[aX11], v2, v22\n\t" \
    "v_fmac_f32 %[aX21], v2, v26\n\t" \
    "s_waitcnt lgkmcnt(0)\n\t" \
    "v_fmac_f32 %[aV02], v5, v17\n\t" \
    "v_fmac_f32 %[aV12], v5, v21\n\t" \
    "v_fmac_f32 %[aV22], v5, v25\n\t" \
    "v_fmac_f32 %[aV02], v4, v16\n\t" \
    "v_fmac_f32 %[aV12], v4, v20\n\t" \
    "v_fmac_f32 %[aV22], v4, v24\n\t" \
    "v_fmac_f32 %[aX02], v7, v19\n\t" \
    "v_fmac_f32 %[aX12], v7, v23\n\t" \
    "v_fmac_f32 %[aX22], v7, v27\n\t" \
    "v_fmac_f32 %[aX02], v6, v18\n\t" \
    "v_fmac_f32 %[aX12], v6, v22\n\t" \
    "v_fmac_f32 %[aX22], v6, v26\n\t" \
    "s_branch .Lkjoin_%=\n\t" \
    ".Lkv4_%=:\n\t" \
    "ds_read_b128 v[0:3], %[fpa] offset:16\n\t" \
    "ds_read_b128 v[4:7], %[fpa] offset:32\n\t" \
    "v_fmac_f32 %[aX00], v49, v17\n\t" \
    "v_fmac_f32 %[aX10], v49, v21\n\t" \
    "v_fmac_f32 %[aX20], v49, v25\n\t" \
    "v_fmac_f32 %[aX00], v48, v16\n\t" \
    "v_fmac_f32 %[aX10], v48, v20\n\t" \
    "v_fmac_f32 %[aX20], v48, v24\n\t" \
    "v_fmac_f32 %[aX00], v51, v19\n\t" \
    "v_fmac_f32 %[aX10], v51, v23\n\t" \
    "v_fmac_f32 %[aX20], v51, v27\n\t" \
    "v_fmac_f32 %[aX00], v50, v18\n\t" \
    "v_fmac_f32 %[aX10], v50, v22\n\t" \
    "v_fmac_f32 %[aX20], v50, v26\n\t" \
    "s_waitcnt lgkmcnt(1)\n\t" \
    "v_fmac_f32 %[aX01], v1, v17\n\t" \
    "v_fmac_f32 %[aX11], v1, v21\n\t" \
    "v_fmac_f32 %[aX21], v1, v25\n\t" \
    "v_fmac_f32 %[aX01], v0, v16\n\t" \
    "v_fmac_f32 %[aX11], v0, v20\n\t" \
    "v_fmac_f32 %[aX21], v0, v24\n\t" \
    "v_fmac_f32 %[aX01], v3, v19\n\t" \
    "v_fmac_f32 %[aX11], v3, v23\n\t" \
    "v_fmac_f32 %[aX21], v3, v27\n\t" \
    "v_fmac_f32 %[aX01], v2, v18\n\t" \
    "v_fmac_f32 %[aX11], v2, v22\n\t" \
    "v_fmac_f32 %[aX21], v2, v26\n\t" \
    "s_waitcnt lgkmcnt(0)\n\t" \
    "v_fmac_f32 %[aX02], v5, v17\n\t" \
    "v_fmac_f32 %[aX12], v5, v21\n\t" \
    "v_fmac_f32 %[aX22], v5, v25\n\t" \
    "v_fmac_f32 %[aX02], v4, v16\n\t" \
    "v_fmac_f32 %[aX12], v4, v20\n\t" \
    "v_fmac_f32 %[aX22], v4, v24\n\t" \
    "v_fmac_f32 %[aX02], v7, v19\n\t" \
    "v_fmac_f32 %[aX12], v7, v23\n\t" \
    "v_fmac_f32 %[aX22], v7, v27\n\t" \
    "v_fmac_f32 %[aX02], v6, v18\n\t" \
    "v_fmac_f32 %[aX12], v6, v22\n\t" \
    "v_fmac_f32 %[aX22], v6, v26\n\t" \
    "s_branch .Lkjoin_%=\n\t" \
    ".Lexit_%=:\n\t" \
    : [D0] "+{v[16:31]}"(D0), [aA0] "+v"(accA[0]), [aA1] "+v"(accA[1]), [aA2] "+v"(accA[2]), [aA3] "+v"(accA[3]), [aV00] "+v"(accV[0][0]), [aX00] "+v"(accX[0][0]), [aV01] "+v"(accV[0][1]), [aX01] "+v"(accX[0][1]), [aV02] "+v"(accV[0][2]), [aX02] "+v"(accX[0][2]), [aV10] "+v"(accV[1][0]), [aX10] "+v"(accX[1][0]), [aV11] "+v"(accV[1][1]), [aX11] "+v"(accX[1][1]), [aV12] "+v"(accV[1][2]), [aX12] "+v"(accX[1][2]), [aV20] "+v"(accV[2][0]), [aX20] "+v"(accX[2][0]), [aV21] "+v"(accV[2][1]), [aX21] "+v"(accX[2][1]), [aV22] "+v"(accV[2][2]), [aX22] "+v"(accX[2][2]), [aV30] "+v"(accV[3][0]), [aX30] "+v"(accX[3][0]), [aV31] "+v"(accV[3][1]), [aX31] "+v"(accX[3][1]), [aV32] "+v"(accV[3][2]), [aX32] "+v"(accX[3][2]), [t0] "=&s"(t0_), [t1] "=&s"(t1_), [t2] "=&s"(t2_), [sel] "=&s"(sel_), [pk0] "=&s"(pk0_), [pk1] "=&s"(pk1_), [pk2] "=&s"(pk2_), [sv] "=&s"(sv_) \
    : [f0] "{v[48:51]}"(f0), [st0] "v"(st0), [st1] "v"(st1), [ringb] "v"(ringb_u), [rw0] "v"(ringw0_u), [rw1] "v"(ringw1_u), [fpa] "v"(fpa_u), [fra] "v"(fra_u), [bsc2] "v"(bsc2), [oscv] "v"(oscv), [s0] "v"(s0), [vx] "v"(vx), [vy] "v"(vy), [vz] "v"(vz), [sm1] "v"(seg.m1), [sm2] "v"(seg.m2), [sm4] "v"(seg.m4), [sm8] "v"(seg.m8), [sm16] "v"(seg.m16), [vrow] "v"(vrow), [hh4] "v"(hh4_u), [hh12] "v"(hh12_u), [w0] "s"(w0), [chan4] "s"(chan4_), [tail] "s"(tail_mask), [sumbase] "s"(sumbase) \
    : "v0", "v1", "v2", "v3", "v4", "v5", "v6", "v7", "v8", "v9", "v10", "v11", "v12", "v13", "v14", "v15", "v52", "v53", "memory", "scc")

#define X3_EPI_2() \
  asm volatile( \
    "ds_read_b128 v[0:3], %[ringb] offset:41760\n\t" \
    "ds_read_b128 v[4:7], %[ringb] offset:41776\n\t" \
    "ds_read_b128 v[8:11], %[ringb] offset:41792\n\t" \
    "ds_read_b128 v[12:15], %[ringb] offset:41808\n\t" \
    "s_waitcnt vmcnt(1)\n\t" \
    "ds_write_b128 %[rw0], %[st0] offset:13968\n\t" \
    "s_waitcnt vmcnt(0)\n\t" \
    "ds_write_b128 %[rw1], %[st1] offset:13968\n\t" \
    "s_waitcnt lgkmcnt(2)\n\t" \
    "v_fmac_f32 v16, v0, %[bsc2]\n\t" \
    "v_fmac_f32 v17, v1, %[bsc2]\n\t" \
    "v_fmac_f32 v18, v2, %[bsc2]\n\t" \
    "v_fmac_f32 v19, v3, %[bsc2]\n\t" \
    "v_fmac_f32 v20, v4, %[bsc2]\n\t" \
    "v_fmac_f32 v21, v5, %[bsc2]\n\t" \
    "v_fmac_f32 v22, v6, %[bsc2]\n\t" \
    "v_fmac_f32 v23, v7, %[bsc2]\n\t" \
    "v_fmac_f32 v24, v8, %[bsc2]\n\t" \
    "v_fmac_f32 v25, v9, %[bsc2]\n\t" \
    "v_fmac_f32 v26, v10, %[bsc2]\n\t" \
    "v_fmac_f32 v27, v11, %[bsc2]\n\t" \
    "v_fmac_f32 v28, v12, %[bsc2]\n\t" \
    "v_fmac_f32 v29, v13, %[bsc2]\n\t" \
    "v_fmac_f32 v30, v14, %[bsc2]\n\t" \
    "v_fmac_f32 v31, v15, %[bsc2]\n\t" \
    "s_and_b32 %[t0], %[w0], 3\n\t" \
    "s_bfe_u32 %[t1], %[w0], 0x2000e\n\t" \
    "s_add_i32 %[t1], %[t1], 3\n\t" \
    "s_add_i32 %[t2], %[t0], 1\n\t" \
    "s_cmp_eq_u32 %[t0], 2\n\t" \
    "s_cselect_b32 %[t2], %[t1], %[t2]\n\t" \
    "s_cmp_eq_u32 %[t0], 3\n\t" \
    "s_cselect_b32 %[sel], 7, %[t2]\n\t" \
    "s_cmp_lg_u32 %[sel], 1\n\t" \
    "s_cbranch_scc1 .Lkrare_%=\n\t" \
    "v_fmac_f32 %[aA0], v51, v19\n\t" \
    "v_fmac_f32 %[aA1], v51, v23\n\t" \
    "v_fmac_f32 %[aA2], v51, v27\n\t" \
    "v_fmac_f32 %[aA3], v51, v31\n\t" \
    "v_fmac_f32 %[aA0], v50, v18\n\t" \
    "v_fmac_f32 %[aA1], v50, v22\n\t" \
    "v_fmac_f32 %[aA2], v50, v26\n\t" \
    "v_fmac_f32 %[aA3], v50, v30\n\t" \
    "v_fmac_f32 %[aA0], v49, v17\n\t" \
    "v_fmac_f32 %[aA1], v49, v21\n\t" \
    "v_fmac_f32 %[aA2], v49, v25\n\t" \
    "v_fmac_f32 %[aA3], v49, v29\n\t" \
    "v_fmac_f32 %[aA0], v48, v16\n\t" \
    "v_fmac_f32 %[aA1], v48, v20\n\t" \
    "v_fmac_f32 %[aA2], v48, v24\n\t" \
    "v_fmac_f32 %[aA3], v48, v28\n\t" \
    ".Lkjoin_%=:\n\t" \
    "s_bitcmp0_b32 %[w0], 7\n\t" \
    "s_cbranch_scc1 .Lnp_%=\n\t" \
    "s_lshr_b32 %[t0], %[w0], 6\n\t" \
    "s_and_b32 %[t0], %[t0], 0xf0\n\t" \
    "v_add_u32 v52, %[t0], %[fra]\n\t" \
    "ds_read_b128 v[8:11], v52\n\t" \
    "s_bfe_u32 %[t1], %[w0], 0x20008\n\t" \
    "s_cmp_eq_u32 %[t1], 0\n\t" \
    "s_cselect_b32 %[pk0], 1.0, 0\n\t" \
    "s_cmp_eq_u32 %[t1], 1\n\t" \
    "s_cselect_b32 %[pk1], 1.0, 0\n\t" \
    "s_cmp_eq_u32 %[t1], 2\n\t" \
    "s_cselect_b32 %[pk2], 1.0, 0\n\t" \
    "s_waitcnt lgkmcnt(0)\n\t" \
    "v_mul_f32 v52, v11, v31\n\t" \
    "v_fmac_f32 v52, v10, v30\n\t" \
    "v_fmac_f32 v52, v9, v29\n\t" \
    "v_fmac_f32 v52, v8, v28\n\t" \
    "v_fmac_f32 %[aA0], %[pk0], v52\n\t" \
    "v_fmac_f32 %[aA1], %[pk1], v52\n\t" \
    "v_fmac_f32 %[aA2], %[pk2], v52\n\t" \
    ".Lnp_%=:\n\t" \
    "s_bfe_u32 %[t0], %[w0], 0x20002\n\t" \
    "s_cmp_eq_u32 %[t0], 0\n\t" \
    "s_cbranch_scc1 .Lnf_%=\n\t" \
    "s_cmp_eq_u32 %[t0], 2\n\t" \
    "s_cbranch_scc1 .Lfv_%=\n\t" \
    "s_cmp_eq_u32 %[sel], 7\n\t" \
    "s_cbranch_scc1 .Lfr_%=\n\t" \
    "v_fma_f32 v0, %[aA0], %[s0], %[aV00]\n\t" \
    "v_fma_f32 v1, %[aA1], %[s0], %[aV10]\n\t" \
    "v_fma_f32 v2, %[aA2], %[s0], %[aV20]\n\t" \
    "v_fma_f32 v3, %[aA3], %[s0], %[aV30]\n\t" \
    "v_mul_f32 v0, %[oscv], v0\n\t" \
    "v_mul_f32 v1, %[oscv], v1\n\t" \
    "v_mul_f32 v2, %[oscv], v2\n\t" \
    "v_mul_f32 v3, %[oscv], v3\n\t" \
    "v_mov_b32 %[aA0], 0\n\t" \
    "v_mov_b32 %[aV00], 0\n\t" \
    "v_mov_b32 %[aA1], 0\n\t" \
// ... 320 lines not shown
    "ds_read_b128 v[0:3], %[fpa] offset:16\n\t" \
    "ds_read_b128 v[4:7], %[fpa] offset:32\n\t" \
    "v_fmac_f32 %[aV00], v49, v17\n\t" \
    "v_fmac_f32 %[aV10], v49, v21\n\t" \
    "v_fmac_f32 %[aV20], v49, v25\n\t" \
    "v_fmac_f32 %[aV00], v48, v16\n\t" \
    "v_fmac_f32 %[aV10], v48, v20\n\t" \
    "v_fmac_f32 %[aV20], v48, v24\n\t" \
    "v_fmac_f32 %[aX00], v51, v19\n\t" \
    "v_fmac_f32 %[aX10], v51, v23\n\t" \
    "v_fmac_f32 %[aX20], v51, v27\n\t" \
    "v_fmac_f32 %[aX00], v50, v18\n\t" \
    "v_fmac_f32 %[aX10], v50, v22\n\t" \
    "v_fmac_f32 %[aX20], v50, v26\n\t" \
    "s_waitcnt lgkmcnt(1)\n\t" \
    "v_fmac_f32 %[aV01], v1, v17\n\t" \
    "v_fmac_f32 %[aV11], v1, v21\n\t" \
    "v_fmac_f32 %[aV21], v1, v25\n\t" \
    "v_fmac_f32 %[aV01], v0, v16\n\t" \
    "v_fmac_f32 %[aV11], v0, v20\n\t" \
    "v_fmac_f32 %[aV21], v0, v24\n\t" \
    "v_fmac_f32 %[aX01], v3, v19\n\t" \
    "v_fmac_f32 %[aX11], v3, v23\n\t" \
    "v_fmac_f32 %[aX21], v3, v27\n\t" \
    "v_fmac_f32 %[aX01], v2, v18\n\t" \
    "v_fmac_f32 %[aX11], v2, v22\n\t" \
    "v_fmac_f32 %[aX21], v2, v26\n\t" \
    "s_waitcnt lgkmcnt(0)\n\t" \
    "v_fmac_f32 %[aV02], v5, v17\n\t" \
    "v_fmac_f32 %[aV12], v5, v21\n\t" \
    "v_fmac_f32 %[aV22], v5, v25\n\t" \
    "v_fmac_f32 %[aV02], v4, v16\n\t" \
    "v_fmac_f32 %[aV12], v4, v20\n\t" \
    "v_fmac_f32 %[aV22], v4, v24\n\t" \
    "v_fmac_f32 %[aX02], v7, v19\n\t" \
    "v_fmac_f32 %[aX12], v7, v23\n\t" \
    "v_fmac_f32 %[aX22], v7, v27\n\t" \
    "v_fmac_f32 %[aX02], v6, v18\n\t" \
    "v_fmac_f32 %[aX12], v6, v22\n\t" \
    "v_fmac_f32 %[aX22], v6, v26\n\t" \
    "s_branch .Lkjoin_%=\n\t" \
    ".Lkv4_%=:\n\t" \
    "ds_read_b128 v[0:3], %[fpa] offset:16\n\t" \
    "ds_read_b128 v[4:7], %[fpa] offset:32\n\t" \
    "v_fmac_f32 %[aX00], v49, v17\n\t" \
    "v_fmac_f32 %[aX10], v49, v21\n\t" \
    "v_fmac_f32 %[aX20], v49, v25\n\t" \
    "v_fmac_f32 %[aX00], v48, v16\n\t" \
    "v_fmac_f32 %[aX10], v48, v20\n\t" \
    "v_fmac_f32 %[aX20], v48, v24\n\t" \
    "v_fmac_f32 %[aX00], v51, v19\n\t" \
    "v_fmac_f32 %[aX10], v51, v23\n\t" \
    "v_fmac_f32 %[aX20], v51, v27\n\t" \
    "v_fmac_f32 %[aX00], v50, v18\n\t" \
    "v_fmac_f32 %[aX10], v50, v22\n\t" \
    "v_fmac_f32 %[aX20], v50, v26\n\t" \
    "s_waitcnt lgkmcnt(1)\n\t" \
    "v_fmac_f32 %[aX01], v1, v17\n\t" \
    "v_fmac_f32 %[aX11], v1, v21\n\t" \
    "v_fmac_f32 %[aX21], v1, v25\n\t" \
    "v_fmac_f32 %[aX01], v0, v16\n\t" \
    "v_fmac_f32 %[aX11], v0, v20\n\t" \
    "v_fmac_f32 %[aX21], v0, v24\n\t" \
    "v_fmac_f32 %[aX01], v3, v19\n\t" \
    "v_fmac_f32 %[aX11], v3, v23\n\t" \
    "v_fmac_f32 %[aX21], v3, v27\n\t" \
    "v_fmac_f32 %[aX01], v2, v18\n\t" \
    "v_fmac_f32 %[aX11], v2, v22\n\t" \
    "v_fmac_f32 %[aX21], v2, v26\n\t" \
    "s_waitcnt lgkmcnt(0)\n\t" \
    "v_fmac_f32 %[aX02], v5, v17\n\t" \
    "v_fmac_f32 %[aX12], v5, v21\n\t" \
    "v_fmac_f32 %[aX22], v5, v25\n\t" \
    "v_fmac_f32 %[aX02], v4, v16\n\t" \
    "v_fmac_f32 %[aX12], v4, v20\n\t" \
    "v_fmac_f32 %[aX22], v4, v24\n\t" \
    "v_fmac_f32 %[aX02], v7, v19\n\t" \
    "v_fmac_f32 %[aX12], v7, v23\n\t" \
    "v_fmac_f32 %[aX22], v7, v27\n\t" \
    "v_fmac_f32 %[aX02], v6, v18\n\t" \
    "v_fmac_f32 %[aX12], v6, v22\n\t" \
    "v_fmac_f32 %[aX22], v6, v26\n\t" \
    "s_branch .Lkjoin_%=\n\t" \
    ".Lexit_%=:\n\t" \
    : [D0] "+{v[16:31]}"(D0), [aA0] "+v"(accA[0]), [aA1] "+v"(accA[1]), [aA2] "+v"(accA[2]), [aA3] "+v"(accA[3]), [aV00] "+v"(accV[0][0]), [aX00] "+v"(accX[0][0]), [aV01] "+v"(accV[0][1]), [aX01] "+v"(accX[0][1]), [aV02] "+v"(accV[0][2]), [aX02] "+v"(accX[0][2]), [aV10] "+v"(accV[1][0]), [aX10] "+v"(accX[1][0]), [aV11] "+v"(accV[1][1]), [aX11] "+v"(accX[1][1]), [aV12] "+v"(accV[1][2]), [aX12] "+v"(accX[1][2]), [aV20] "+v"(accV[2][0]), [aX20] "+v"(accX[2][0]), [aV21] "+v"(accV[2][1]), [aX21] "+v"(accX[2][1]), [aV22] "+v"(accV[2][2]), [aX22] "+v"(accX[2][2]), [aV30] "+v"(accV[3][0]), [aX30] "+v"(accX[3][0]), [aV31] "+v"(accV[3][1]), [aX31] "+v"(accX[3][1]), [aV32] "+v"(accV[3][2]), [aX32] "+v"(accX[3][2]), [t0] "=&s"(t0_), [t1] "=&s"(t1_), [t2] "=&s"(t2_), [sel] "=&s"(sel_), [pk0] "=&s"(pk0_), [pk1] "=&s"(pk1_), [pk2] "=&s"(pk2_), [sv] "=&s"(sv_) \
    : [f0] "{v[48:51]}"(f0), [st0] "v"(st0), [st1] "v"(st1), [ringb] "v"(ringb_u), [rw0] "v"(ringw0_u), [rw1] "v"(ringw1_u), [fpa] "v"(fpa_u), [fra] "v"(fra_u), [bsc2] "v"(bsc2), [oscv] "v"(oscv), [s0] "v"(s0), [vx] "v"(vx), [vy] "v"(vy), [vz] "v"(vz), [sm1] "v"(seg.m1), [sm2] "v"(seg.m2), [sm4] "v"(seg.m4), [sm8] "v"(seg.m8), [sm16] "v"(seg.m16), [vrow] "v"(vrow), [hh4] "v"(hh4_u), [hh12] "v"(hh12_u), [w0] "s"(w0), [chan4] "s"(chan4_), [tail] "s"(tail_mask), [sumbase] "s"(sumbase) \
    : "v0", "v1", "v2", "v3", "v4", "v5", "v6", "v7", "v8", "v9", "v10", "v11", "v12", "v13", "v14", "v15", "v52", "v53", "memory", "scc")

#define X3_EPI_3() \
  asm volatile( \
    "ds_read_b128 v[0:3], %[ringb] offset:55728\n\t" \
    "ds_read_b128 v[4:7], %[ringb] offset:55744\n\t" \
    "ds_read_b128 v[8:11], %[ringb] offset:55760\n\t" \
    "ds_read_b128 v[12:15], %[ringb] offset:55776\n\t" \
    "s_waitcnt vmcnt(1)\n\t" \
    "ds_write_b128 %[rw0], %[st0] offset:27936\n\t" \
    "s_waitcnt vmcnt(0)\n\t" \
    "ds_write_b128 %[rw1], %[st1] offset:27936\n\t" \
    "s_waitcnt lgkmcnt(2)\n\t" \
    "v_fmac_f32 v16, v0, %[bsc2]\n\t" \
    "v_fmac_f32 v17, v1, %[bsc2]\n\t" \
    "v_fmac_f32 v18, v2, %[bsc2]\n\t" \
    "v_fmac_f32 v19, v3, %[bsc2]\n\t" \
    "v_fmac_f32 v20, v4, %[bsc2]\n\t" \
    "v_fmac_f32 v21, v5, %[bsc2]\n\t" \
    "v_fmac_f32 v22, v6, %[bsc2]\n\t" \
    "v_fmac_f32 v23, v7, %[bsc2]\n\t" \
    "v_fmac_f32 v24, v8, %[bsc2]\n\t" \
    "v_fmac_f32 v25, v9, %[bsc2]\n\t" \
    "v_fmac_f32 v26, v10, %[bsc2]\n\t" \
    "v_fmac_f32 v27, v11, %[bsc2]\n\t" \
    "v_fmac_f32 v28, v12, %[bsc2]\n\t" \
    "v_fmac_f32 v29, v13, %[bsc2]\n\t" \
    "v_fmac_f32 v30, v14, %[bsc2]\n\t" \
    "v_fmac_f32 v31, v15, %[bsc2]\n\t" \
    "s_and_b32 %[t0], %[w0], 3\n\t" \
    "s_bfe_u32 %[t1], %[w0], 0x2000e\n\t" \
    "s_add_i32 %[t1], %[t1], 3\n\t" \
    "s_add_i32 %[t2], %[t0], 1\n\t" \
    "s_cmp_eq_u32 %[t0], 2\n\t" \
    "s_cselect_b32 %[t2], %[t1], %[t2]\n\t" \
    "s_cmp_eq_u32 %[t0], 3\n\t" \
    "s_cselect_b32 %[sel], 7, %[t2]\n\t" \
    "s_cmp_lg_u32 %[sel], 1\n\t" \
    "s_cbranch_scc1 .Lkrare_%=\n\t" \
    "v_fmac_f32 %[aA0], v51, v19\n\t" \
    "v_fmac_f32 %[aA1], v51, v23\n\t" \
    "v_fmac_f32 %[aA2], v51, v27\n\t" \
    "v_fmac_f32 %[aA3], v51, v31\n\t" \
    "v_fmac_f32 %[aA0], v50, v18\n\t" \
    "v_fmac_f32 %[aA1], v50, v22\n\t" \
    "v_fmac_f32 %[aA2], v50, v26\n\t" \
    "v_fmac_f32 %[aA3], v50, v30\n\t" \
    "v_fmac_f32 %[aA0], v49, v17\n\t" \
    "v_fmac_f32 %[aA1], v49, v21\n\t" \
    "v_fmac_f32 %[aA2], v49, v25\n\t" \
    "v_fmac_f32 %[aA3], v49, v29\n\t" \
    "v_fmac_f32 %[aA0], v48, v16\n\t" \
    "v_fmac_f32 %[aA1], v48, v20\n\t" \
    "v_fmac_f32 %[aA2], v48, v24\n\t" \
    "v_fmac_f32 %[aA3], v48, v28\n\t" \
    ".Lkjoin_%=:\n\t" \
    "s_bitcmp0_b32 %[w0], 7\n\t" \
    "s_cbranch_scc1 .Lnp_%=\n\t" \
    "s_lshr_b32 %[t0], %[w0], 6\n\t" \
    "s_and_b32 %[t0], %[t0], 0xf0\n\t" \
    "v_add_u32 v52, %[t0], %[fra]\n\t" \
    "ds_read_b128 v[8:11], v52\n\t" \
    "s_bfe_u32 %[t1], %[w0], 0x20008\n\t" \
    "s_cmp_eq_u32 %[t1], 0\n\t" \
    "s_cselect_b32 %[pk0], 1.0, 0\n\t" \
    "s_cmp_eq_u32 %[t1], 1\n\t" \
    "s_cselect_b32 %[pk1], 1.0, 0\n\t" \
    "s_cmp_eq_u32 %[t1], 2\n\t" \
    "s_cselect_b32 %[pk2], 1.0, 0\n\t" \
    "s_waitcnt lgkmcnt(0)\n\t" \
    "v_mul_f32 v52, v11, v31\n\t" \
    "v_fmac_f32 v52, v10, v30\n\t" \
    "v_fmac_f32 v52, v9, v29\n\t" \
    "v_fmac_f32 v52, v8, v28\n\t" \
    "v_fmac_f32 %[aA0], %[pk0], v52\n\t" \
    "v_fmac_f32 %[aA1], %[pk1], v52\n\t" \
    "v_fmac_f32 %[aA2], %[pk2], v52\n\t" \
    ".Lnp_%=:\n\t" \
    "s_bfe_u32 %[t0], %[w0], 0x20002\n\t" \
    "s_cmp_eq_u32 %[t0], 0\n\t" \
    "s_cbranch_scc1 .Lnf_%=\n\t" \
    "s_cmp_eq_u32 %[t0], 2\n\t" \
    "s_cbranch_scc1 .Lfv_%=\n\t" \
    "s_cmp_eq_u32 %[sel], 7\n\t" \
    "s_cbranch_scc1 .Lfr_%=\n\t" \
    "v_fma_f32 v0, %[aA0], %[s0], %[aV00]\n\t" \
    "v_fma_f32 v1, %[aA1], %[s0], %[aV10]\n\t" \
    "v_fma_f32 v2, %[aA2], %[s0], %[aV20]\n\t" \
    "v_fma_f32 v3, %[aA3], %[s0], %[aV30]\n\t" \
    "v_mul_f32 v0, %[oscv], v0\n\t" \
    "v_mul_f32 v1, %[oscv], v1\n\t" \
    "v_mul_f32 v2, %[oscv], v2\n\t" \
    "v_mul_f32 v3, %[oscv], v3\n\t" \
    "v_mov_b32 %[aA0], 0\n\t" \
    "v_mov_b32 %[aV00], 0\n\t" \
    "v_mov_b32 %[aA1], 0\n\t" \
// ... 320 lines not shown
    "ds_read_b128 v[0:3], %[fpa] offset:16\n\t" \
    "ds_read_b128 v[4:7], %[fpa] offset:32\n\t" \
    "v_fmac_f32 %[aV00], v49, v17\n\t" \
    "v_fmac_f32 %[aV10], v49, v21\n\t" \
    "v_fmac_f32 %[aV20], v49, v25\n\t" \
    "v_fmac_f32 %[aV00], v48, v16\n\t" \
    "v_fmac_f32 %[aV10], v48, v20\n\t" \
    "v_fmac_f32 %[aV20], v48, v24\n\t" \
    "v_fmac_f32 %[aX00], v51, v19\n\t" \
    "v_fmac_f32 %[aX10], v51, v23\n\t" \
    "v_fmac_f32 %[aX20], v51, v27\n\t" \
    "v_fmac_f32 %[aX00], v50, v18\n\t" \
    "v_fmac_f32 %[aX10], v50, v22\n\t" \
    "v_fmac_f32 %[aX20], v50, v26\n\t" \
    "s_waitcnt lgkmcnt(1)\n\t" \
    "v_fmac_f32 %[aV01], v1, v17\n\t" \
    "v_fmac_f32 %[aV11], v1, v21\n\t" \
    "v_fmac_f32 %[aV21], v1, v25\n\t" \
    "v_fmac_f32 %[aV01], v0, v16\n\t" \
    "v_fmac_f32 %[aV11], v0, v20\n\t" \
    "v_fmac_f32 %[aV21], v0, v24\n\t" \
    "v_fmac_f32 %[aX01], v3, v19\n\t" \
    "v_fmac_f32 %[aX11], v3, v23\n\t" \
    "v_fmac_f32 %[aX21], v3, v27\n\t" \
    "v_fmac_f32 %[aX01], v2, v18\n\t" \
    "v_fmac_f32 %[aX11], v2, v22\n\t" \
    "v_fmac_f32 %[aX21], v2, v26\n\t" \
    "s_waitcnt lgkmcnt(0)\n\t" \
    "v_fmac_f32 %[aV02], v5, v17\n\t" \
    "v_fmac_f32 %[aV12], v5, v21\n\t" \
    "v_fmac_f32 %[aV22], v5, v25\n\t" \
    "v_fmac_f32 %[aV02], v4, v16\n\t" \
    "v_fmac_f32 %[aV12], v4, v20\n\t" \
    "v_fmac_f32 %[aV22], v4, v24\n\t" \
    "v_fmac_f32 %[aX02], v7, v19\n\t" \
    "v_fmac_f32 %[aX12], v7, v23\n\t" \
    "v_fmac_f32 %[aX22], v7, v27\n\t" \
    "v_fmac_f32 %[aX02], v6, v18\n\t" \
    "v_fmac_f32 %[aX12], v6, v22\n\t" \
    "v_fmac_f32 %[aX22], v6, v26\n\t" \
    "s_branch .Lkjoin_%=\n\t" \
    ".Lkv4_%=:\n\t" \
    "ds_read_b128 v[0:3], %[fpa] offset:16\n\t" \
    "ds_read_b128 v[4:7], %[fpa] offset:32\n\t" \
    "v_fmac_f32 %[aX00], v49, v17\n\t" \
    "v_fmac_f32 %[aX10], v49, v21\n\t" \
    "v_fmac_f32 %[aX20], v49, v25\n\t" \
    "v_fmac_f32 %[aX00], v48, v16\n\t" \
    "v_fmac_f32 %[aX10], v48, v20\n\t" \
    "v_fmac_f32 %[aX20], v48, v24\n\t" \
    "v_fmac_f32 %[aX00], v51, v19\n\t" \
    "v_fmac_f32 %[aX10], v51, v23\n\t" \
    "v_fmac_f32 %[aX20], v51, v27\n\t" \
    "v_fmac_f32 %[aX00], v50, v18\n\t" \
    "v_fmac_f32 %[aX10], v50, v22\n\t" \
    "v_fmac_f32 %[aX20], v50, v26\n\t" \
    "s_waitcnt lgkmcnt(1)\n\t" \
    "v_fmac_f32 %[aX01], v1, v17\n\t" \
    "v_fmac_f32 %[aX11], v1, v21\n\t" \
    "v_fmac_f32 %[aX21], v1, v25\n\t" \
    "v_fmac_f32 %[aX01], v0, v16\n\t" \
    "v_fmac_f32 %[aX11], v0, v20\n\t" \
    "v_fmac_f32 %[aX21], v0, v24\n\t" \
    "v_fmac_f32 %[aX01], v3, v19\n\t" \
    "v_fmac_f32 %[aX11], v3, v23\n\t" \
    "v_fmac_f32 %[aX21], v3, v27\n\t" \
    "v_fmac_f32 %[aX01], v2, v18\n\t" \
    "v_fmac_f32 %[aX11], v2, v22\n\t" \
    "v_fmac_f32 %[aX21], v2, v26\n\t" \
    "s_waitcnt lgkmcnt(0)\n\t" \
    "v_fmac_f32 %[aX02], v5, v17\n\t" \
    "v_fmac_f32 %[aX12], v5, v21\n\t" \
    "v_fmac_f32 %[aX22], v5, v25\n\t" \
    "v_fmac_f32 %[aX02], v4, v16\n\t" \
    "v_fmac_f32 %[aX12], v4, v20\n\t" \
    "v_fmac_f32 %[aX22], v4, v24\n\t" \
    "v_fmac_f32 %[aX02], v7, v19\n\t" \
    "v_fmac_f32 %[aX12], v7, v23\n\t" \
    "v_fmac_f32 %[aX22], v7, v27\n\t" \
    "v_fmac_f32 %[aX02], v6, v18\n\t" \
    "v_fmac_f32 %[aX12], v6, v22\n\t" \
    "v_fmac_f32 %[aX22], v6, v26\n\t" \
    "s_branch .Lkjoin_%=\n\t" \
    ".Lexit_%=:\n\t" \
    : [D0] "+{v[16:31]}"(D0), [aA0] "+v"(accA[0]), [aA1] "+v"(accA[1]), [aA2] "+v"(accA[2]), [aA3] "+v"(accA[3]), [aV00] "+v"(accV[0][0]), [aX00] "+v"(accX[0][0]), [aV01] "+v"(accV[0][1]), [aX01] "+v"(accX[0][1]), [aV02] "+v"(accV[0][2]), [aX02] "+v"(accX[0][2]), [aV10] "+v"(accV[1][0]), [aX10] "+v"(accX[1][0]), [aV11] "+v"(accV[1][1]), [aX11] "+v"(accX[1][1]), [aV12] "+v"(accV[1][2]), [aX12] "+v"(accX[1][2]), [aV20] "+v"(accV[2][0]), [aX20] "+v"(accX[2][0]), [aV21] "+v"(accV[2][1]), [aX21] "+v"(accX[2][1]), [aV22] "+v"(accV[2][2]), [aX22] "+v"(accX[2][2]), [aV30] "+v"(accV[3][0]), [aX30] "+v"(accX[3][0]), [aV31] "+v"(accV[3][1]), [aX31] "+v"(accX[3][1]), [aV32] "+v"(accV[3][2]), [aX32] "+v"(accX[3][2]), [t0] "=&s"(t0_), [t1] "=&s"(t1_), [t2] "=&s"(t2_), [sel] "=&s"(sel_), [pk0] "=&s"(pk0_), [pk1] "=&s"(pk1_), [pk2] "=&s"(pk2_), [sv] "=&s"(sv_) \
    : [f0] "{v[48:51]}"(f0), [st0] "v"(st0), [st1] "v"(st1), [ringb] "v"(ringb_u), [rw0] "v"(ringw0_u), [rw1] "v"(ringw1_u), [fpa] "v"(fpa_u), [fra] "v"(fra_u), [bsc2] "v"(bsc2), [oscv] "v"(oscv), [s0] "v"(s0), [vx] "v"(vx), [vy] "v"(vy), [vz] "v"(vz), [sm1] "v"(seg.m1), [sm2] "v"(seg.m2), [sm4] "v"(seg.m4), [sm8] "v"(seg.m8), [sm16] "v"(seg.m16), [vrow] "v"(vrow), [hh4] "v"(hh4_u), [hh12] "v"(hh12_u), [w0] "s"(w0), [chan4] "s"(chan4_), [tail] "s"(tail_mask), [sumbase] "s"(sumbase) \
    : "v0", "v1", "v2", "v3", "v4", "v5", "v6", "v7", "v8", "v9", "v10", "v11", "v12", "v13", "v14", "v15", "v52", "v53", "memory", "scc")
```

Measured before the change: 48.78.

## Pack two-limb conv weights compactly and stage first-layer weights in LDS

In two-limb mode, conv weight records are packed without the unused third fp16 limb, which shrinks each W2 tile record and the W1 tiles. The split-mode first-layer weights are copied into an LDS area once per weight group and read from there instead of global memory. The ring prefetch and the hand-written epilogue assembly are changed to the smaller record size, with the second copy chunk masked by a ballot. This reduces global and LDS traffic per tile, at the cost of an extra block barrier whenever the weight group changes and new LDS offsets in the assembly.

```diff
diff --git a/disco_diffdock_amd/csrc/ddk_capi.hip b/disco_diffdock_amd/csrc/ddk_capi.hip
--- a/disco_diffdock_amd/csrc/ddk_capi.hip
+++ b/disco_diffdock_amd/csrc/ddk_capi.hip
@@ -346,15 +346,23 @@
 static int pack_x3(ddk_ctx* ctx, ConvLayerDev& L, int NG, const std::vector<float>& w1all, const std::vector<float>& w2all,
                    const std::vector<float>& b2all) {
   const size_t w1sz = 3 * 9 * 64 * 4, w2sz = (size_t)L.n_tiles * 9 * 64 * 4, b2sz = (size_t)L.n_tiles * 32;
+  const int limbs = ctx->cfg.conv_kernel == 3 ? 3 : 2;
+  const int tile_bytes = limbs == 3 ? W2X_TILE_BYTES : W2X2_TILE_BYTES, bias_off = limbs == 3 ? W2X_BIAS_OFF : W2X2_BIAS_OFF,
+            desc_off = limbs == 3 ? W2X_DESC_OFF : W2X2_DESC_OFF, w1_tile_bytes = limbs == 3 ? W1X_TILE_BYTES : W1X2_TILE_BYTES;
   bool exact = true;
-  auto split = [&exact](float v, uint16_t& hi, uint16_t& mid, uint16_t& lo) {
+  auto split = [&exact, limbs](float v, uint16_t& hi, uint16_t& mid, uint16_t& lo) {
     const _Float16 h = (_Float16)v;
     const float r1 = v - (float)h;
     const _Float16 m = (_Float16)r1;
     const _Float16 l = (_Float16)(r1 - (float)m);
     memcpy(&hi, &h, 2); memcpy(&mid, &m, 2); memcpy(&lo, &l, 2);
-    const double back = (double)(float)h + (double)(float)m + (double)(float)l;
-    if (std::fabs(v) >= 0.5f ? back != (double)v : std::fabs(back - (double)v) > 0x1p-25) exact = false;
+    if (limbs == 3) {
+      const double back = (double)(float)h + (double)(float)m + (double)(float)l;
+      if (std::fabs(v) >= 0.5f ? back != (double)v : std::fabs(back - (double)v) > 0x1p-25) exact = false;
+    } else {
+      const double back = (double)(float)h + (double)(float)m;
+      if (std::fabs(back - (double)v) > std::max(0x1p-22 * std::fabs((double)v), 0x1p-25)) exact = false;
+    }
   };
   auto range_scale = [](const float* v, size_t n, const float* v2, size_t n2) {
     float m = 0.f;
@@ -364,7 +372,7 @@
     std::frexp(std::max(m, 0x1p-40f), &e);
     return std::ldexp(1.0f, 15 - e);
   };
-  std::vector<uint8_t> w2x((size_t)(NG * L.n_tiles + 4) * W2X_TILE_BYTES, 0), w1x((size_t)NG * 3 * W1X_TILE_BYTES, 0);
+  std::vector<uint8_t> w2x((size_t)(NG * L.n_tiles + 4) * tile_bytes, 0), w1x((size_t)NG * 3 * w1_tile_bytes, 0);
   auto frags = [&](const float* src, float sc, uint8_t* dst) {
     for (int r = 0; r < 36; ++r)
       for (int lane = 0; lane < 64; ++lane) {
@@ -373,7 +381,8 @@
         const size_t off = s_ < 4 ? (size_t)s_ * 1024 + lane * 16 + 2 * i : (size_t)4096 + lane * 8 + 2 * i;
         uint16_t h, m, l;
         split(v, h, m, l);
-        memcpy(dst + off, &h, 2); memcpy(dst + W2X_LIMB_BYTES + off, &m, 2); memcpy(dst + 2 * W2X_LIMB_BYTES + off, &l, 2);
+        memcpy(dst + off, &h, 2); memcpy(dst + W2X_LIMB_BYTES + off, &m, 2);
+        if (limbs == 3) memcpy(dst + 2 * W2X_LIMB_BYTES + off, &l, 2);
       }
   };
   for (int g = 0; g < NG; ++g) {
@@ -383,26 +392,28 @@
     const float sc1 = range_scale(w1, w1sz, nullptr, 0), sc2 = range_scale(w2, w2sz, nullptr, 0);
     L.w1s[g] = sc1; L.w2s[g] = sc2;
     for (int t = 0; t < L.n_tiles; ++t) {
-      uint8_t* rec = w2x.data() + ((size_t)g * L.n_tiles + t) * W2X_TILE_BYTES;
+      uint8_t* rec = w2x.data() + ((size_t)g * L.n_tiles + t) * tile_bytes;
       frags(w2 + (size_t)t * 2304, sc2, rec);
-      memcpy(rec + W2X_BIAS_OFF, b2 + (size_t)t * 32, 128);
+      memcpy(rec + bias_off, b2 + (size_t)t * 32, 128);
       const int32_t dq[2] = {x_tile_word(L.h_tiles[t].w0), L.h_tiles[t].chan0};
       if (dq[0] < 0) return fail(ctx, DDK_ERR_INVALID, "internal: a vector tile of the conv layout does not sit on a T1O / T1E row quad");
-      memcpy(rec + W2X_DESC_OFF, dq, 8);
-    }
-    for (int T = 0; T < 3; ++T) frags(w1 + (size_t)T * 2304, sc1, w1x.data() + ((size_t)g * 3 + T) * W1X_TILE_BYTES);
-  }
-  if (!exact) return fail(ctx, DDK_ERR_INVALID, "internal: the three-limb fp16 split of a conv weight is not exact");
+      memcpy(rec + desc_off, dq, 8);
+    }
+    for (int T = 0; T < 3; ++T) frags(w1 + (size_t)T * 2304, sc1, w1x.data() + ((size_t)g * 3 + T) * w1_tile_bytes);
+  }
+  if (!exact)
+    return fail(ctx, DDK_ERR_INVALID, limbs == 3 ? "internal: the three-limb fp16 split of a conv weight is not exact"
+                                                 : "internal: the two-limb fp16 split of a conv weight leaves its 2^-22 window");
   L.h_w2x = w2x; L.h_w1x = w1x;
   L.epi_ok = conv_epilogue_shapes_ok(L.h_tiles);
-  L.limbs = ctx->cfg.conv_kernel == 3 ? 3 : 2;
+  L.limbs = limbs;
   if (ctx->host_only) return DDK_OK;
   L.w2x = (uint8_t*)dev_alloc(ctx, w2x.size());
   L.w1x = (uint8_t*)dev_alloc(ctx, w1x.size());
-  if (!L.w2x || !L.w1x) return fail(ctx, DDK_ERR_NOMEM, "device allocation failed while packing conv weights (three-limb f16)");
+  if (!L.w2x || !L.w1x) return fail(ctx, DDK_ERR_NOMEM, "device allocation failed while packing conv weights (f16 limbs)");
   if (hipMemcpy(L.w2x, w2x.data(), w2x.size(), hipMemcpyHostToDevice) != hipSuccess ||
       hipMemcpy(L.w1x, w1x.data(), w1x.size(), hipMemcpyHostToDevice) != hipSuccess)
-    return fail(ctx, DDK_ERR_HIP, "three-limb weight upload failed");
+    return fail(ctx, DDK_ERR_HIP, "f16-limb weight upload failed");
   return DDK_OK;
 }
 
diff --git a/disco_diffdock_amd/csrc/ddk_internal.h b/disco_diffdock_amd/csrc/ddk_internal.h
--- a/disco_diffdock_amd/csrc/ddk_internal.h
+++ b/disco_diffdock_amd/csrc/ddk_internal.h
@@ -49,12 +49,20 @@
 constexpr int W2X_DESC_OFF = W2X_BIAS_OFF + 128;
 constexpr int W2X_TILE_BYTES = W2X_DESC_OFF + 16;
 constexpr int W1X_TILE_BYTES = 3 * W2X_LIMB_BYTES;
+constexpr int W2X2_BIAS_OFF = 2 * W2X_LIMB_BYTES;
+constexpr int W2X2_DESC_OFF = W2X2_BIAS_OFF + 128;
+constexpr int W2X2_TILE_BYTES = W2X2_DESC_OFF + 16;
+constexpr int W1X2_TILE_BYTES = 2 * W2X_LIMB_BYTES;
+constexpr int W1L_LIMB_BYTES = 1024 + 512;
+constexpr int W1L_BYTES = 3 * 2 * W1L_LIMB_BYTES;
 constexpr int CONV_TRACE_TILES = 1024;
 constexpr int FX_A = 0, FX_C = NS, FX_R = 2 * NS, FX_PQ = FX_R + 6 * NV, FX_STRIDE = FX_PQ + 12 + 4;
 static_assert(FX_STRIDE == 100 && FX_A == F_A && FX_C == F_C, "F row layout (three-limb f16)");
 constexpr int W2X_STAGES = 4;
 constexpr size_t CONV_X_LDS_BYTES = (size_t)CONV_WAVES * 32 * FX_STRIDE * 4 + W2X_STAGES * W2X_TILE_BYTES + 16;
 static_assert(CONV_X_LDS_BYTES <= 160 * 1024 && W2X_TILE_BYTES % 16 == 0, "LDS budget (three-limb f16)");
+constexpr size_t CONV_X2_LDS_BYTES = (size_t)CONV_WAVES * 32 * FX_STRIDE * 4 + W2X_STAGES * W2X2_TILE_BYTES + W1L_BYTES + 16;
+static_assert(CONV_X2_LDS_BYTES <= 160 * 1024 && W2X2_TILE_BYTES % 16 == 0 && W1L_BYTES % 16 == 0, "LDS budget (two-limb f16)");
 
 enum TileKind : int {
   T_RA = 0,
diff --git a/disco_diffdock_amd/csrc/k_conv_x.hip b/disco_diffdock_amd/csrc/k_conv_x.hip
--- a/disco_diffdock_amd/csrc/k_conv_x.hip
+++ b/disco_diffdock_amd/csrc/k_conv_x.hip
@@ -7,6 +7,13 @@
 #define launch_conv_fused_x launch_conv_fused_x2
 #define conv_prepare_device_x conv_prepare_device_x2
 #include "k_conv_x_epi2_gen.inc"
+#define X3_TILE_BYTES W2X2_TILE_BYTES
+#define X3_BIAS_OFF W2X2_BIAS_OFF
+#define X3_DESC_OFF W2X2_DESC_OFF
+#define X3_W1_TILE_BYTES W1X2_TILE_BYTES
+#define X3_LDS_BYTES CONV_X2_LDS_BYTES
+#define X3_W1L_BYTES W1L_BYTES
+#define X3_TWO true
 #define X3_SUM(r) D0[r]
 #define X3_TAIL3(a_lh, a_hm) (void)(a_lh); D0 = MFMA16(a_hm, HT.mh, D0); D0 = MFMA16(a_hm, HT.hm, D0);
 #define X3_STEP(MF, ah, am, al, bh, bm, bl)   \
@@ -24,6 +31,13 @@
 #define X3_TAIL_BARES X3_BARE X3_BARE
 #else
 #include "k_conv_x_epi_gen.inc"
+#define X3_TILE_BYTES W2X_TILE_BYTES
+#define X3_BIAS_OFF W2X_BIAS_OFF
+#define X3_DESC_OFF W2X_DESC_OFF
+#define X3_W1_TILE_BYTES W1X_TILE_BYTES
+#define X3_LDS_BYTES CONV_X_LDS_BYTES
+#define X3_W1L_BYTES 0
+#define X3_TWO false
 #define X3_SUM(r) (D0[r] + D1[r])
 #define X3_TAIL3(a_lh, a_hm) D0 = MFMA16(a_hm, HT.mh, D0); D1 = MFMA16(a_lh, HT.hl, D1); D0 = MFMA16(a_hm, HT.hm, D0);
 #define X3_STEP(MF, ah, am, al, bh, bm, bl)   \
@@ -50,6 +64,34 @@
 #define MFMA16(a, b, c) __builtin_amdgcn_mfma_f32_32x32x16_f16((a), (b), (c), 0, 0, 0)
 #define MFMA8(a, b, c) __builtin_amdgcn_mfma_f32_32x32x8f16((a), (b), (c), 0, 0, 0)
 
+struct W1Split { f16x8 h, m, l; f16x4 th, tm, tl; };
+#ifdef X3_TWO_LIMBS
+template <class TY> __device__ __forceinline__ TY w1_lo(const char*, const TY& hi) { return hi; }
+__device__ __forceinline__ W1Split w1_split(const char* w1l, const char*, int T, int lane) {
+  const char* wt = w1l + T * (2 * W1L_LIMB_BYTES);
+  W1Split f;
+  f.h = *reinterpret_cast<const f16x8*>(wt + lane * 16);
+  f.m = *reinterpret_cast<const f16x8*>(wt + W1L_LIMB_BYTES + lane * 16);
+  f.th = *reinterpret_cast<const f16x4*>(wt + 1024 + lane * 8);
+  f.tm = *reinterpret_cast<const f16x4*>(wt + W1L_LIMB_BYTES + 1024 + lane * 8);
+  f.l = f.h; f.tl = f.th;
+  return f;
+}
+#else
+template <class TY> __device__ __forceinline__ TY w1_lo(const char* p, const TY&) { return *reinterpret_cast<const TY*>(p); }
+__device__ __forceinline__ W1Split w1_split(const char*, const char* w1, int T, int lane) {
+  const char* wt = w1 + (size_t)T * W1X_TILE_BYTES;
+  W1Split f;
+  f.h = *reinterpret_cast<const f16x8*>(wt + lane * 16);
+  f.m = *reinterpret_cast<const f16x8*>(wt + W2X_LIMB_BYTES + lane * 16);
+  f.l = *reinterpret_cast<const f16x8*>(wt + 2 * W2X_LIMB_BYTES + lane * 16);
+  f.th = *reinterpret_cast<const f16x4*>(wt + 1024 + lane * 16);
+  f.tm = *reinterpret_cast<const f16x4*>(wt + W2X_LIMB_BYTES + 1024 + lane * 16);
+  f.tl = *reinterpret_cast<const f16x4*>(wt + 2 * W2X_LIMB_BYTES + 1024 + lane * 16);
+  return f;
+}
+#endif
+
 __device__ __forceinline__ float range_scale(float m, float& inv) {
   const uint32_t eb = max((__float_as_uint(m) >> 23) & 0xffu, 87u);
   inv = __uint_as_float((eb - 14u) << 23);
@@ -225,7 +267,9 @@
   const int tid = threadIdx.x, lane = tid & 63, wave = tid >> 6;
   float* F = lds + wave * (32 * FS);
   char* ring = reinterpret_cast<char*>(lds + WAVES * (32 * FS));
-  int* blk_slot = reinterpret_cast<int*>(ring + W2X_STAGES * W2X_TILE_BYTES);
+  char* w1l = ring + W2X_STAGES * X3_TILE_BYTES;
+  int* blk_slot = reinterpret_cast<int*>(w1l + X3_W1L_BYTES);
+  (void)w1l;
   const int el = lane & 31;
   const int hh = lane >> 5;
   const bool g2_shared = A.sum_g2 != nullptr;
@@ -249,9 +293,15 @@
   float* Fr = F + el * FS;
   const float inv_s3 = 0.57735026918962576451f, inv_s2 = 0.70710678118654752440f;
   const int n_tiles = A.n_tiles;
-  constexpr int REC16 = W2X_TILE_BYTES / 16;
+  constexpr int REC16 = X3_TILE_BYTES / 16;
   const int grp = wave >> 2;
   const uint32_t fo0 = 16u * tid, fo1 = 16u * min(tid + 64 * WAVES, REC16 - 1);
+  const bool has1 = !X3_TWO || tid + 64 * WAVES < REC16;
+  const unsigned long long c1_mask = __ballot(has1);
+  const bool has1_s = !X3_TWO || c1_mask != 0;
+  (void)has1; (void)has1_s; (void)c1_mask;
+  int gw_lds = -1;
+  (void)gw_lds;
   constexpr bool ASM_EPI = GATHER && SPLIT && !DET && MODE == 0;
   const unsigned ring0_u = (unsigned)(WAVES * 32 * FS * 4), ringb_u = ring0_u + 64u * hh, ringw0_u = ring0_u + fo0, ringw1_u = ring0_u + fo1;
   const unsigned fra_u = (unsigned)((wave * 32 + el) * FS * 4), hh4_u = 4u * hh, hh12_u = 12u * hh;
@@ -302,21 +352,42 @@
     const int sn = A.src[e], dn = A.dst[e];
 
     const int gw = (int)((A.wmap >> (4 * g)) & 15);
-    const char* wrec = reinterpret_cast<const char*>(A.w2x) + (size_t)gw * n_tiles * W2X_TILE_BYTES;
+    const char* wrec = reinterpret_cast<const char*>(A.w2x) + (size_t)gw * n_tiles * X3_TILE_BYTES;
     {
-      const char* wr0 = wrec + (size_t)t_begin * W2X_TILE_BYTES;
-      const char* wr1 = wrec + (size_t)min(t_begin + 1, t_end - 1) * W2X_TILE_BYTES;
-      const char* wr2 = wrec + (size_t)min(t_begin + 2, t_end - 1) * W2X_TILE_BYTES;
-      const float4 r0 = *reinterpret_cast<const float4*>(wr0 + fo0), r1 = *reinterpret_cast<const float4*>(wr0 + fo1);
-      const float4 r2 = *reinterpret_cast<const float4*>(wr1 + fo0), r3 = *reinterpret_cast<const float4*>(wr1 + fo1);
-      const float4 r4 = *reinterpret_cast<const float4*>(wr2 + fo0), r5 = *reinterpret_cast<const float4*>(wr2 + fo1);
+      const char* wr0 = wrec + (size_t)t_begin * X3_TILE_BYTES;
+      const char* wr1 = wrec + (size_t)min(t_begin + 1, t_end - 1) * X3_TILE_BYTES;
+      const char* wr2 = wrec + (size_t)min(t_begin + 2, t_end - 1) * X3_TILE_BYTES;
+      const float4 r0 = *reinterpret_cast<const float4*>(wr0 + fo0);
+      const float4 r2 = *reinterpret_cast<const float4*>(wr1 + fo0);
+      const float4 r4 = *reinterpret_cast<const float4*>(wr2 + fo0);
+      if (has1_s) { if (has1) {
+        const float4 r1 = *reinterpret_cast<const float4*>(wr0 + fo1);
+        const float4 r3 = *reinterpret_cast<const float4*>(wr1 + fo1);
+        const float4 r5 = *reinterpret_cast<const float4*>(wr2 + fo1);
+        *reinterpret_cast<float4*>(ring + fo1) = r1;
+        *reinterpret_cast<float4*>(ring + X3_TILE_BYTES + fo1) = r3;
+        *reinterpret_cast<float4*>(ring + 2 * X3_TILE_BYTES + fo1) = r5;
+      } }
       *reinterpret_cast<float4*>(ring + fo0) = r0;
-      *reinterpret_cast<float4*>(ring + fo1) = r1;
-      *reinterpret_cast<float4*>(ring + W2X_TILE_BYTES + fo0) = r2;
-      *reinterpret_cast<float4*>(ring + W2X_TILE_BYTES + fo1) = r3;
-      *reinterpret_cast<float4*>(ring + 2 * W2X_TILE_BYTES + fo0) = r4;
-      *reinterpret_cast<float4*>(ring + 2 * W2X_TILE_BYTES + fo1) = r5;
-    }
+      *reinterpret_cast<float4*>(ring + X3_TILE_BYTES + fo0) = r2;
+      *reinterpret_cast<float4*>(ring + 2 * X3_TILE_BYTES + fo0) = r4;
+    }
+#ifdef X3_TWO_LIMBS
+    if constexpr (SPLIT) {
+      const int gw_s = __builtin_amdgcn_readfirstlane(gw);
+      if (gw_s != gw_lds) {
+        if (wave < 6) {
+          const char* wsrc = reinterpret_cast<const char*>(A.w1x) + ((size_t)gw_s * 3 + (wave >> 1)) * X3_W1_TILE_BYTES + (wave & 1) * W2X_LIMB_BYTES;
+          const float4 c16 = *reinterpret_cast<const float4*>(wsrc + lane * 16);
+          const float2 c8 = *reinterpret_cast<const float2*>(wsrc + 1024 + lane * 16);
+          *reinterpret_cast<float4*>(w1l + wave * W1L_LIMB_BYTES + lane * 16) = c16;
+          *reinterpret_cast<float2*>(w1l + wave * W1L_LIMB_BYTES + 1024 + lane * 8) = c8;
+        }
+        gw_lds = gw_s;
+        lds_barrier();
+      }
+    }
+#endif
 
     const SegF seg = make_segf(make_segctl(sn, el, nvalid, valid));
     stamp(5);
@@ -337,7 +408,8 @@
     float osc, bsc2;
     {
       float h[36];
-      const char* w1 = reinterpret_cast<const char*>(A.w1x) + (size_t)gw * 3 * W1X_TILE_BYTES;
+      const char* w1 = reinterpret_cast<const char*>(A.w1x) + (size_t)gw * 3 * X3_W1_TILE_BYTES;
+      (void)w1;
       if constexpr (SPLIT) {
         float4 psv[9], pdv[9];
         {
@@ -384,17 +456,10 @@
           }
 #pragma unroll
           for (int r = 0; r < 16; ++r) D1[r] = 0.0f;
-          const char* wt = w1 + (size_t)T * W1X_TILE_BYTES;
+          const W1Split wf = w1_split(w1l, w1, T, lane);
+          X3_STEP(MFMA16, wf.h, wf.m, wf.l, b0h, b0m, b0l)
           {
-            const f16x8 ah = *reinterpret_cast<const f16x8*>(wt + lane * 16);
-            const f16x8 am = *reinterpret_cast<const f16x8*>(wt + W2X_LIMB_BYTES + lane * 16);
-            const f16x8 al = *reinterpret_cast<const f16x8*>(wt + 2 * W2X_LIMB_BYTES + lane * 16);
-            X3_STEP(MFMA16, ah, am, al, b0h, b0m, b0l)
-          }
-          {
-            const f16x4 ah = *reinterpret_cast<const f16x4*>(wt + 1024 + lane * 16);
-            const f16x4 am = *reinterpret_cast<const f16x4*>(wt + W2X_LIMB_BYTES + 1024 + lane * 16);
-            const f16x4 al = *reinterpret_cast<const f16x4*>(wt + 2 * W2X_LIMB_BYTES + 1024 + lane * 16);
+            const f16x4 ah = wf.th, am = wf.tm, al = wf.tl;
             const f16x8 a_hm = __builtin_shufflevector(ah, am, 0, 1, 2, 3, 4, 5, 6, 7), a_lh = __builtin_shufflevector(al, ah, 0, 1, 2, 3, 4, 5, 6, 7);
             D0 = MFMA16(a_hm, b1_mh, D0);
 #ifndef X3_TWO_LIMBS
@@ -451,18 +516,18 @@
           }
 #pragma unroll
           for (int r = 0; r < 16; ++r) D1[r] = 0.0f;
-          const char* wt = w1 + (size_t)T * W1X_TILE_BYTES;
+          const char* wt = w1 + (size_t)T * X3_W1_TILE_BYTES;
 #pragma unroll
           for (int s = 0; s < 4; ++s) {
             const f16x8 ah = *reinterpret_cast<const f16x8*>(wt + s * 1024 + lane * 16);
             const f16x8 am = *reinterpret_cast<const f16x8*>(wt + W2X_LIMB_BYTES + s * 1024 + lane * 16);
-            const f16x8 al = *reinterpret_cast<const f16x8*>(wt + 2 * W2X_LIMB_BYTES + s * 1024 + lane * 16);
+            const f16x8 al = w1_lo<f16x8>(wt + 2 * W2X_LIMB_BYTES + s * 1024 + lane * 16, ah);
             X3_STEP(MFMA16, ah, am, al, Bn.hi[s], Bn.mid[s], Bn.lo[s])
           }
           {
             const f16x4 ah = *reinterpret_cast<const f16x4*>(wt + 4096 + lane * 8);
             const f16x4 am = *reinterpret_cast<const f16x4*>(wt + W2X_LIMB_BYTES + 4096 + lane * 8);
-            const f16x4 al = *reinterpret_cast<const f16x4*>(wt + 2 * W2X_LIMB_BYTES + 4096 + lane * 8);
+            const f16x4 al = w1_lo<f16x4>(wt + 2 * W2X_LIMB_BYTES + 4096 + lane * 8, ah);
             X3_STEP(MFMA8, ah, am, al, Bn.thi, Bn.tmid, Bn.tlo)
           }
           const int nr = T < 2 ? 16 : 4;
@@ -538,7 +603,7 @@
     char* ringw0 = ring + fo0;
     char* ringw1 = ring + fo1;
     const __amdgpu_buffer_rsrc_t rsrc = __builtin_amdgcn_make_buffer_rsrc(const_cast<char*>(wrec), 0, 0x7fffffff, 0x00020000);
-    int rec_soff = (t_begin + 3) * W2X_TILE_BYTES;
+    int rec_soff = (t_begin + 3) * X3_TILE_BYTES;
     Frag16 p0;
     p0.h = *reinterpret_cast<const f16x8*>(ringl); p0.m = *reinterpret_cast<const f16x8*>(ringl + W2X_LIMB_BYTES);
 #ifndef X3_TWO_LIMBS
@@ -546,7 +611,7 @@
 #endif
     int w0, chan0;
     {
-      const int2 dq = *reinterpret_cast<const int2*>(ring + W2X_DESC_OFF);
+      const int2 dq = *reinterpret_cast<const int2*>(ring + X3_DESC_OFF);
       w0 = __builtin_amdgcn_readfirstlane(dq.x); chan0 = __builtin_amdgcn_readfirstlane(dq.y);
     }
     const bool grp_s = __builtin_amdgcn_readfirstlane(grp) != 0;
@@ -601,10 +666,10 @@
 #define X3_BURST_BODY(ST)                                                                                                                    \
       Frag16 p1; X3_FRAG(p1, SO + 1024)                                                                                                      \
       const f32x4 f0 = ldv4(Fp);                                                                                                             \
-                                    \
+            \
       const u32x4 st0 = __builtin_amdgcn_raw_buffer_load_b128(rsrc, (int)fo0, rec_soff, 0);                                                  \
-      const u32x4 st1 = __builtin_amdgcn_raw_buffer_load_b128(rsrc, (int)fo1, rec_soff, 0);                                                  \
-      rec_soff += W2X_TILE_BYTES;                                                                                                            \
+      if constexpr (!X3_TWO) st1 = __builtin_amdgcn_raw_buffer_load_b128(rsrc, (int)fo1, rec_soff, 0);                                      \
+      rec_soff += X3_TILE_BYTES;                                                                                                             \
       X3_STEP(MFMA16, p0.h, p0.m, p0.l, H.hi[0], H.mid[0], H.lo[0])                                                                         \
       X3_RIDERS_0                                                                                                                            \
       __builtin_amdgcn_sched_barrier(0);                                                                                                     \
@@ -619,17 +684,23 @@
       X3_STEP(MFMA16, q2.h, q2.m, q2.l, H.hi[2], H.mid[2], H.lo[2])                                                                         \
       X3_RIDERS_2                                                                                                                            \
       __builtin_amdgcn_sched_barrier(0);                                                                                                     \
-      const int2 dq = *reinterpret_cast<const int2*>(ring + SN + W2X_DESC_OFF);                                                              \
+      const int2 dq = *reinterpret_cast<const int2*>(ring + SN + X3_DESC_OFF);                                                               \
       X3_FRAG(p0, SN)           \
       X3_STEP(MFMA16, q3.h, q3.m, q3.l, H.hi[3], H.mid[3], H.lo[3])                                                                         \
       X3_RIDERS_3                                                                                                                            \
       __builtin_amdgcn_sched_barrier(0);
 #define X3_TILE(ST)                                                                                                                          \
     {                                                                                                                                        \
-      constexpr int SO = (ST) * W2X_TILE_BYTES, SN = (((ST) + 1) & 3) * W2X_TILE_BYTES, SW = (((ST) + 3) & 3) * W2X_TILE_BYTES;              \
+      constexpr int SO = (ST) * X3_TILE_BYTES, SN = (((ST) + 1) & 3) * X3_TILE_BYTES, SW = (((ST) + 3) & 3) * X3_TILE_BYTES;                 \
                       \
       __builtin_amdgcn_s_setprio(1);                                                                                                         \
       stamp(0);                                                                                                                              \
+                                                                   \
+      u32x4 st1;                                                                                                                             \
+      if constexpr (X3_TWO) {                                                                                                                \
+        asm volatile("" : "=v"(st1));                                                                                                        \
+        if (has1_s) { if (has1) st1 = __builtin_amdgcn_raw_buffer_load_b128(rsrc, (int)fo1, rec_soff, 0); }                                  \
+      }                                                                                                                                      \
                                                         \
       const float* Fp = Fr + ((w0 >> 16) & 0xff);                                                                                            \
       f32x16 D0, D1;                                                                                                                         \
@@ -652,10 +723,12 @@
         const int chan4_ = chan0 * 4;                                                                                                        \
         X3_EPI_##ST();                                                                                                                       \
       } else {                                                                                                                               \
-      const float4 bs0 = ld4(reinterpret_cast<const float*>(ringb + SO + W2X_BIAS_OFF)), bs1 = ld4(reinterpret_cast<const float*>(ringb + SO + W2X_BIAS_OFF + 16)); \
-      const float4 bs2 = ld4(reinterpret_cast<const float*>(ringb + SO + W2X_BIAS_OFF + 32)), bs3 = ld4(reinterpret_cast<const float*>(ringb + SO + W2X_BIAS_OFF + 48)); \
+       \
+      if constexpr (X3_TWO) { if (has1_s) { if (has1) *reinterpret_cast<u32x4*>(ringw1 + SW) = st1; } }                                      \
+      const float4 bs0 = ld4(reinterpret_cast<const float*>(ringb + SO + X3_BIAS_OFF)), bs1 = ld4(reinterpret_cast<const float*>(ringb + SO + X3_BIAS_OFF + 16)); \
+      const float4 bs2 = ld4(reinterpret_cast<const float*>(ringb + SO + X3_BIAS_OFF + 32)), bs3 = ld4(reinterpret_cast<const float*>(ringb + SO + X3_BIAS_OFF + 48)); \
       *reinterpret_cast<u32x4*>(ringw0 + SW) = st0;                                                                                          \
-      *reinterpret_cast<u32x4*>(ringw1 + SW) = st1;                                                                                          \
+      if constexpr (!X3_TWO) *reinterpret_cast<u32x4*>(ringw1 + SW) = st1;                                                                   \
                                                                                              \
       D0[0] = fmaf(bs0.x, bsc2, X3_SUM(0)); D0[1] = fmaf(bs0.y, bsc2, X3_SUM(1)); D0[2] = fmaf(bs0.z, bsc2, X3_SUM(2)); D0[3] = fmaf(bs0.w, bsc2, X3_SUM(3)); \
       D0[4] = fmaf(bs1.x, bsc2, X3_SUM(4)); D0[5] = fmaf(bs1.y, bsc2, X3_SUM(5)); D0[6] = fmaf(bs1.z, bsc2, X3_SUM(6)); D0[7] = fmaf(bs1.w, bsc2, X3_SUM(7)); \
@@ -726,14 +799,14 @@
 
 template <bool GATHER, bool SPLIT, bool DET>
 static hipError_t launch_x_t(const ConvXArgs& k, int n_cu, hipStream_t s) {
-  hipLaunchKernelGGL((conv_x3_kernel<GATHER, SPLIT, DET>), dim3(n_cu), dim3(64 * CONV_WAVES), CONV_X_LDS_BYTES, s, k);
+  hipLaunchKernelGGL((conv_x3_kernel<GATHER, SPLIT, DET>), dim3(n_cu), dim3(64 * CONV_WAVES), X3_LDS_BYTES, s, k);
   return hipGetLastError();
 }
 
 template <bool GATHER, bool SPLIT, bool DET>
 static hipError_t attr_x_t() {
   return hipFuncSetAttribute(reinterpret_cast<const void*>(&conv_x3_kernel<GATHER, SPLIT, DET>), hipFuncAttributeMaxDynamicSharedMemorySize,
-                             (int)CONV_X_LDS_BYTES);
+                             (int)X3_LDS_BYTES);
 }
 
 #ifndef X3_TWO_LIMBS
@@ -760,13 +833,13 @@
   if (e == hipSuccess) e = attr_x_t<false, false, true>();
   if (e == hipSuccess)
     e = hipFuncSetAttribute(reinterpret_cast<const void*>(&conv_x3_kernel<true, true, false, true>), hipFuncAttributeMaxDynamicSharedMemorySize,
-                            (int)CONV_X_LDS_BYTES);
+                            (int)X3_LDS_BYTES);
   if (e == hipSuccess)
     e = hipFuncSetAttribute(reinterpret_cast<const void*>(&conv_x3_kernel<true, false, false, false, 1>), hipFuncAttributeMaxDynamicSharedMemorySize,
-                            (int)CONV_X_LDS_BYTES);
+                            (int)X3_LDS_BYTES);
   if (e == hipSuccess)
     e = hipFuncSetAttribute(reinterpret_cast<const void*>(&conv_x3_kernel<false, false, false, false, 1>), hipFuncAttributeMaxDynamicSharedMemorySize,
-                            (int)CONV_X_LDS_BYTES);
+                            (int)X3_LDS_BYTES);
   return e;
 }
 
@@ -790,8 +863,8 @@
   X.trace = nullptr; X.trace_coarse = a.trace_coarse;
   if (a.mode == 1) {
     if (a.pre != nullptr || a.part != nullptr || a.trace != nullptr) return hipErrorInvalidValue;
-    if (a.gather) hipLaunchKernelGGL((conv_x3_kernel<true, false, false, false, 1>), dim3(n_cu), dim3(64 * CONV_WAVES), CONV_X_LDS_BYTES, s, X);
-    else hipLaunchKernelGGL((conv_x3_kernel<false, false, false, false, 1>), dim3(n_cu), dim3(64 * CONV_WAVES), CONV_X_LDS_BYTES, s, X);
+    if (a.gather) hipLaunchKernelGGL((conv_x3_kernel<true, false, false, false, 1>), dim3(n_cu), dim3(64 * CONV_WAVES), X3_LDS_BYTES, s, X);
+    else hipLaunchKernelGGL((conv_x3_kernel<false, false, false, false, 1>), dim3(n_cu), dim3(64 * CONV_WAVES), X3_LDS_BYTES, s, X);
     return hipGetLastError();
   }
   if (a.part != nullptr) {
@@ -805,7 +878,7 @@
   X.trace = a.trace;
   if (a.trace != nullptr) {
     if (!(a.gather && a.pre != nullptr)) return hipErrorInvalidValue;
-    hipLaunchKernelGGL((conv_x3_kernel<true, true, false, true>), dim3(n_cu), dim3(64 * CONV_WAVES), CONV_X_LDS_BYTES, s, X);
+    hipLaunchKernelGGL((conv_x3_kernel<true, true, false, true>), dim3(n_cu), dim3(64 * CONV_WAVES), X3_LDS_BYTES, s, X);
     return hipGetLastError();
   }
   if (a.gather && a.pre != nullptr) return launch_x_t<true, true, false>(X, n_cu, s);
diff --git a/disco_diffdock_amd/csrc/k_conv_x_epi2_gen.inc b/disco_diffdock_amd/csrc/k_conv_x_epi2_gen.inc
--- a/disco_diffdock_amd/csrc/k_conv_x_epi2_gen.inc
+++ b/disco_diffdock_amd/csrc/k_conv_x_epi2_gen.inc
@@ -1,15 +1,16 @@
 
 #define X3_EPI_0() \
   asm volatile( \
-    "ds_read_b128 v[0:3], %[ringb] offset:13824\n\t" \
-    "ds_read_b128 v[4:7], %[ringb] offset:13840\n\t" \
-    "ds_read_b128 v[8:11], %[ringb] offset:13856\n\t" \
-    "ds_read_b128 v[12:15], %[ringb] offset:13872\n\t" \
-    "s_waitcnt vmcnt(1)\n\t" \
-    "ds_write_b128 %[rw0], %[st0] offset:41904\n\t" \
+    "ds_read_b128 v[0:3], %[ringb] offset:9216\n\t" \
+    "ds_read_b128 v[4:7], %[ringb] offset:9232\n\t" \
+    "ds_read_b128 v[8:11], %[ringb] offset:9248\n\t" \
+    "ds_read_b128 v[12:15], %[ringb] offset:9264\n\t" \
+    "s_cmp_lg_u64 %[c1], 0\n\t" \
+    "s_cbranch_scc1 .Lr2_%=\n\t" \
     "s_waitcnt vmcnt(0)\n\t" \
-    "ds_write_b128 %[rw1], %[st1] offset:41904\n\t" \
-    "s_waitcnt lgkmcnt(2)\n\t" \
+    "ds_write_b128 %[rw0], %[st0] offset:28080\n\t" \
+    "s_waitcnt lgkmcnt(1)\n\t" \
+    ".Lrj_%=:\n\t" \
     "v_fmac_f32 v16, v0, %[bsc2]\n\t" \
     "v_fmac_f32 v17, v1, %[bsc2]\n\t" \
     "v_fmac_f32 v18, v2, %[bsc2]\n\t" \
@@ -496,22 +497,29 @@
     "v_fmac_f32 %[aX12], v6, v22\n\t" \
     "v_fmac_f32 %[aX22], v6, v26\n\t" \
     "s_branch .Lkjoin_%=\n\t" \
+    ".Lr2_%=:\n\t" \
+    "s_waitcnt vmcnt(0)\n\t" \
+    "ds_write_b128 %[rw0], %[st0] offset:28080\n\t" \
+    "s_mov_b64 %[sv], exec\n\ts_and_b64 exec, exec, %[c1]\n\tds_write_b128 %[rw1], %[st1] offset:28080\n\ts_mov_b64 exec, %[sv]\n\t" \
+    "s_waitcnt lgkmcnt(2)\n\t" \
+    "s_branch .Lrj_%=\n\t" \
     ".Lexit_%=:\n\t" \
     : [D0] "+{v[16:31]}"(D0), [aA0] "+v"(accA[0]), [aA1] "+v"(accA[1]), [aA2] "+v"(accA[2]), [aA3] "+v"(accA[3]), [aV00] "+v"(accV[0][0]), [aX00] "+v"(accX[0][0]), [aV01] "+v"(accV[0][1]), [aX01] "+v"(accX[0][1]), [aV02] "+v"(accV[0][2]), [aX02] "+v"(accX[0][2]), [aV10] "+v"(accV[1][0]), [aX10] "+v"(accX[1][0]), [aV11] "+v"(accV[1][1]), [aX11] "+v"(accX[1][1]), [aV12] "+v"(accV[1][2]), [aX12] "+v"(accX[1][2]), [aV20] "+v"(accV[2][0]), [aX20] "+v"(accX[2][0]), [aV21] "+v"(accV[2][1]), [aX21] "+v"(accX[2][1]), [aV22] "+v"(accV[2][2]), [aX22] "+v"(accX[2][2]), [aV30] "+v"(accV[3][0]), [aX30] "+v"(accX[3][0]), [aV31] "+v"(accV[3][1]), [aX31] "+v"(accX[3][1]), [aV32] "+v"(accV[3][2]), [aX32] "+v"(accX[3][2]), [t0] "=&s"(t0_), [t1] "=&s"(t1_), [t2] "=&s"(t2_), [sel] "=&s"(sel_), [pk0] "=&s"(pk0_), [pk1] "=&s"(pk1_), [pk2] "=&s"(pk2_), [sv] "=&s"(sv_) \
-    : [f0] "{v[48:51]}"(f0), [st0] "v"(st0), [st1] "v"(st1), [ringb] "v"(ringb_u), [rw0] "v"(ringw0_u), [rw1] "v"(ringw1_u), [fpa] "v"(fpa_u), [fra] "v"(fra_u), [bsc2] "v"(bsc2), [oscv] "v"(oscv), [s0] "v"(s0), [vx] "v"(vx), [vy] "v"(vy), [vz] "v"(vz), [sm1] "v"(seg.m1), [sm2] "v"(seg.m2), [sm4] "v"(seg.m4), [sm8] "v"(seg.m8), [sm16] "v"(seg.m16), [vrow] "v"(vrow), [hh4] "v"(hh4_u), [hh12] "v"(hh12_u), [w0] "s"(w0), [chan4] "s"(chan4_), [tail] "s"(tail_mask), [sumbase] "s"(sumbase) \
+    : [f0] "{v[48:51]}"(f0), [st0] "v"(st0), [st1] "v"(st1), [ringb] "v"(ringb_u), [rw0] "v"(ringw0_u), [rw1] "v"(ringw1_u), [fpa] "v"(fpa_u), [fra] "v"(fra_u), [bsc2] "v"(bsc2), [oscv] "v"(oscv), [s0] "v"(s0), [vx] "v"(vx), [vy] "v"(vy), [vz] "v"(vz), [sm1] "v"(seg.m1), [sm2] "v"(seg.m2), [sm4] "v"(seg.m4), [sm8] "v"(seg.m8), [sm16] "v"(seg.m16), [vrow] "v"(vrow), [hh4] "v"(hh4_u), [hh12] "v"(hh12_u), [w0] "s"(w0), [chan4] "s"(chan4_), [tail] "s"(tail_mask), [sumbase] "s"(sumbase), [c1] "s"(c1_mask) \
     : "v0", "v1", "v2", "v3", "v4", "v5", "v6", "v7", "v8", "v9", "v10", "v11", "v12", "v13", "v14", "v15", "v52", "v53", "memory", "scc")
 
 #define X3_EPI_1() \
   asm volatile( \
-    "ds_read_b128 v[0:3], %[ringb] offset:27792\n\t" \
-    "ds_read_b128 v[4:7], %[ringb] offset:27808\n\t" \
-    "ds_read_b128 v[8:11], %[ringb] offset:27824\n\t" \
-    "ds_read_b128 v[12:15], %[ringb] offset:27840\n\t" \
-    "s_waitcnt vmcnt(1)\n\t" \
+    "ds_read_b128 v[0:3], %[ringb] offset:18576\n\t" \
+    "ds_read_b128 v[4:7], %[ringb] offset:18592\n\t" \
+    "ds_read_b128 v[8:11], %[ringb] offset:18608\n\t" \
+    "ds_read_b128 v[12:15], %[ringb] offset:18624\n\t" \
+    "s_cmp_lg_u64 %[c1], 0\n\t" \
+    "s_cbranch_scc1 .Lr2_%=\n\t" \
+    "s_waitcnt vmcnt(0)\n\t" \
     "ds_write_b128 %[rw0], %[st0] offset:0\n\t" \
-    "s_waitcnt vmcnt(0)\n\t" \
-    "ds_write_b128 %[rw1], %[st1] offset:0\n\t" \
-    "s_waitcnt lgkmcnt(2)\n\t" \
+    "s_waitcnt lgkmcnt(1)\n\t" \
+    ".Lrj_%=:\n\t" \
     "v_fmac_f32 v16, v0, %[bsc2]\n\t" \
     "v_fmac_f32 v17, v1, %[bsc2]\n\t" \
     "v_fmac_f32 v18, v2, %[bsc2]\n\t" \
@@ -998,22 +1006,29 @@
     "v_fmac_f32 %[aX12], v6, v22\n\t" \
     "v_fmac_f32 %[aX22], v6, v26\n\t" \
     "s_branch .Lkjoin_%=\n\t" \
+    ".Lr2_%=:\n\t" \
+    "s_waitcnt vmcnt(0)\n\t" \
+    "ds_write_b128 %[rw0], %[st0] offset:0\n\t" \
+    "s_mov_b64 %[sv], exec\n\ts_and_b64 exec, exec, %[c1]\n\tds_write_b128 %[rw1], %[st1] offset:0\n\ts_mov_b64 exec, %[sv]\n\t" \
+    "s_waitcnt lgkmcnt(2)\n\t" \
+    "s_branch .Lrj_%=\n\t" \
     ".Lexit_%=:\n\t" \
     : [D0] "+{v[16:31]}"(D0), [aA0] "+v"(accA[0]), [aA1] "+v"(accA[1]), [aA2] "+v"(accA[2]), [aA3] "+v"(accA[3]), [aV00] "+v"(accV[0][0]), [aX00] "+v"(accX[0][0]), [aV01] "+v"(accV[0][1]), [aX01] "+v"(accX[0][1]), [aV02] "+v"(accV[0][2]), [aX02] "+v"(accX[0][2]), [aV10] "+v"(accV[1][0]), [aX10] "+v"(accX[1][0]), [aV11] "+v"(accV[1][1]), [aX11] "+v"(accX[1][1]), [aV12] "+v"(accV[1][2]), [aX12] "+v"(accX[1][2]), [aV20] "+v"(accV[2][0]), [aX20] "+v"(accX[2][0]), [aV21] "+v"(accV[2][1]), [aX21] "+v"(accX[2][1]), [aV22] "+v"(accV[2][2]), [aX22] "+v"(accX[2][2]), [aV30] "+v"(accV[3][0]), [aX30] "+v"(accX[3][0]), [aV31] "+v"(accV[3][1]), [aX31] "+v"(accX[3][1]), [aV32] "+v"(accV[3][2]), [aX32] "+v"(accX[3][2]), [t0] "=&s"(t0_), [t1] "=&s"(t1_), [t2] "=&s"(t2_), [sel] "=&s"(sel_), [pk0] "=&s"(pk0_), [pk1] "=&s"(pk1_), [pk2] "=&s"(pk2_), [sv] "=&s"(sv_) \
-    : [f0] "{v[48:51]}"(f0), [st0] "v"(st0), [st1] "v"(st1), [ringb] "v"(ringb_u), [rw0] "v"(ringw0_u), [rw1] "v"(ringw1_u), [fpa] "v"(fpa_u), [fra] "v"(fra_u), [bsc2] "v"(bsc2), [oscv] "v"(oscv), [s0] "v"(s0), [vx] "v"(vx), [vy] "v"(vy), [vz] "v"(vz), [sm1] "v"(seg.m1), [sm2] "v"(seg.m2), [sm4] "v"(seg.m4), [sm8] "v"(seg.m8), [sm16] "v"(seg.m16), [vrow] "v"(vrow), [hh4] "v"(hh4_u), [hh12] "v"(hh12_u), [w0] "s"(w0), [chan4] "s"(chan4_), [tail] "s"(tail_mask), [sumbase] "s"(sumbase) \
+    : [f0] "{v[48:51]}"(f0), [st0] "v"(st0), [st1] "v"(st1), [ringb] "v"(ringb_u), [rw0] "v"(ringw0_u), [rw1] "v"(ringw1_u), [fpa] "v"(fpa_u), [fra] "v"(fra_u), [bsc2] "v"(bsc2), [oscv] "v"(oscv), [s0] "v"(s0), [vx] "v"(vx), [vy] "v"(vy), [vz] "v"(vz), [sm1] "v"(seg.m1), [sm2] "v"(seg.m2), [sm4] "v"(seg.m4), [sm8] "v"(seg.m8), [sm16] "v"(seg.m16), [vrow] "v"(vrow), [hh4] "v"(hh4_u), [hh12] "v"(hh12_u), [w0] "s"(w0), [chan4] "s"(chan4_), [tail] "s"(tail_mask), [sumbase] "s"(sumbase), [c1] "s"(c1_mask) \
     : "v0", "v1", "v2", "v3", "v4", "v5", "v6", "v7", "v8", "v9", "v10", "v11", "v12", "v13", "v14", "v15", "v52", "v53", "memory", "scc")
 
 #define X3_EPI_2() \
   asm volatile( \
-    "ds_read_b128 v[0:3], %[ringb] offset:41760\n\t" \
-    "ds_read_b128 v[4:7], %[ringb] offset:41776\n\t" \
-    "ds_read_b128 v[8:11], %[ringb] offset:41792\n\t" \
-    "ds_read_b128 v[12:15], %[ringb] offset:41808\n\t" \
-    "s_waitcnt vmcnt(1)\n\t" \
-    "ds_write_b128 %[rw0], %[st0] offset:13968\n\t" \
+    "ds_read_b128 v[0:3], %[ringb] offset:27936\n\t" \
+    "ds_read_b128 v[4:7], %[ringb] offset:27952\n\t" \
+    "ds_read_b128 v[8:11], %[ringb] offset:27968\n\t" \
+    "ds_read_b128 v[12:15], %[ringb] offset:27984\n\t" \
+    "s_cmp_lg_u64 %[c1], 0\n\t" \
+    "s_cbranch_scc1 .Lr2_%=\n\t" \
     "s_waitcnt vmcnt(0)\n\t" \
-    "ds_write_b128 %[rw1], %[st1] offset:13968\n\t" \
-    "s_waitcnt lgkmcnt(2)\n\t" \
+    "ds_write_b128 %[rw0], %[st0] offset:9360\n\t" \
+    "s_waitcnt lgkmcnt(1)\n\t" \
+    ".Lrj_%=:\n\t" \
     "v_fmac_f32 v16, v0, %[bsc2]\n\t" \
     "v_fmac_f32 v17, v1, %[bsc2]\n\t" \
     "v_fmac_f32 v18, v2, %[bsc2]\n\t" \
@@ -1500,22 +1515,29 @@
     "v_fmac_f32 %[aX12], v6, v22\n\t" \
     "v_fmac_f32 %[aX22], v6, v26\n\t" \
     "s_branch .Lkjoin_%=\n\t" \
+    ".Lr2_%=:\n\t" \
+    "s_waitcnt vmcnt(0)\n\t" \
+    "ds_write_b128 %[rw0], %[st0] offset:9360\n\t" \
+    "s_mov_b64 %[sv], exec\n\ts_and_b64 exec, exec, %[c1]\n\tds_write_b128 %[rw1], %[st1] offset:9360\n\ts_mov_b64 exec, %[sv]\n\t" \
+    "s_waitcnt lgkmcnt(2)\n\t" \
+    "s_branch .Lrj_%=\n\t" \
     ".Lexit_%=:\n\t" \
     : [D0] "+{v[16:31]}"(D0), [aA0] "+v"(accA[0]), [aA1] "+v"(accA[1]), [aA2] "+v"(accA[2]), [aA3] "+v"(accA[3]), [aV00] "+v"(accV[0][0]), [aX00] "+v"(accX[0][0]), [aV01] "+v"(accV[0][1]), [aX01] "+v"(accX[0][1]), [aV02] "+v"(accV[0][2]), [aX02] "+v"(accX[0][2]), [aV10] "+v"(accV[1][0]), [aX10] "+v"(accX[1][0]), [aV11] "+v"(accV[1][1]), [aX11] "+v"(accX[1][1]), [aV12] "+v"(accV[1][2]), [aX12] "+v"(accX[1][2]), [aV20] "+v"(accV[2][0]), [aX20] "+v"(accX[2][0]), [aV21] "+v"(accV[2][1]), [aX21] "+v"(accX[2][1]), [aV22] "+v"(accV[2][2]), [aX22] "+v"(accX[2][2]), [aV30] "+v"(accV[3][0]), [aX30] "+v"(accX[3][0]), [aV31] "+v"(accV[3][1]), [aX31] "+v"(accX[3][1]), [aV32] "+v"(accV[3][2]), [aX32] "+v"(accX[3][2]), [t0] "=&s"(t0_), [t1] "=&s"(t1_), [t2] "=&s"(t2_), [sel] "=&s"(sel_), [pk0] "=&s"(pk0_), [pk1] "=&s"(pk1_), [pk2] "=&s"(pk2_), [sv] "=&s"(sv_) \
-    : [f0] "{v[48:51]}"(f0), [st0] "v"(st0), [st1] "v"(st1), [ringb] "v"(ringb_u), [rw0] "v"(ringw0_u), [rw1] "v"(ringw1_u), [fpa] "v"(fpa_u), [fra] "v"(fra_u), [bsc2] "v"(bsc2), [oscv] "v"(oscv), [s0] "v"(s0), [vx] "v"(vx), [vy] "v"(vy), [vz] "v"(vz), [sm1] "v"(seg.m1), [sm2] "v"(seg.m2), [sm4] "v"(seg.m4), [sm8] "v"(seg.m8), [sm16] "v"(seg.m16), [vrow] "v"(vrow), [hh4] "v"(hh4_u), [hh12] "v"(hh12_u), [w0] "s"(w0), [chan4] "s"(chan4_), [tail] "s"(tail_mask), [sumbase] "s"(sumbase) \
+    : [f0] "{v[48:51]}"(f0), [st0] "v"(st0), [st1] "v"(st1), [ringb] "v"(ringb_u), [rw0] "v"(ringw0_u), [rw1] "v"(ringw1_u), [fpa] "v"(fpa_u), [fra] "v"(fra_u), [bsc2] "v"(bsc2), [oscv] "v"(oscv), [s0] "v"(s0), [vx] "v"(vx), [vy] "v"(vy), [vz] "v"(vz), [sm1] "v"(seg.m1), [sm2] "v"(seg.m2), [sm4] "v"(seg.m4), [sm8] "v"(seg.m8), [sm16] "v"(seg.m16), [vrow] "v"(vrow), [hh4] "v"(hh4_u), [hh12] "v"(hh12_u), [w0] "s"(w0), [chan4] "s"(chan4_), [tail] "s"(tail_mask), [sumbase] "s"(sumbase), [c1] "s"(c1_mask) \
     : "v0", "v1", "v2", "v3", "v4", "v5", "v6", "v7", "v8", "v9", "v10", "v11", "v12", "v13", "v14", "v15", "v52", "v53", "memory", "scc")
 
 #define X3_EPI_3() \
   asm volatile( \
-    "ds_read_b128 v[0:3], %[ringb] offset:55728\n\t" \
-    "ds_read_b128 v[4:7], %[ringb] offset:55744\n\t" \
-    "ds_read_b128 v[8:11], %[ringb] offset:55760\n\t" \
-    "ds_read_b128 v[12:15], %[ringb] offset:55776\n\t" \
-    "s_waitcnt vmcnt(1)\n\t" \
-    "ds_write_b128 %[rw0], %[st0] offset:27936\n\t" \
+    "ds_read_b128 v[0:3], %[ringb] offset:37296\n\t" \
+    "ds_read_b128 v[4:7], %[ringb] offset:37312\n\t" \
+    "ds_read_b128 v[8:11], %[ringb] offset:37328\n\t" \
+    "ds_read_b128 v[12:15], %[ringb] offset:37344\n\t" \
+    "s_cmp_lg_u64 %[c1], 0\n\t" \
+    "s_cbranch_scc1 .Lr2_%=\n\t" \
     "s_waitcnt vmcnt(0)\n\t" \
-    "ds_write_b128 %[rw1], %[st1] offset:27936\n\t" \
-    "s_waitcnt lgkmcnt(2)\n\t" \
+    "ds_write_b128 %[rw0], %[st0] offset:18720\n\t" \
+    "s_waitcnt lgkmcnt(1)\n\t" \
+    ".Lrj_%=:\n\t" \
     "v_fmac_f32 v16, v0, %[bsc2]\n\t" \
     "v_fmac_f32 v17, v1, %[bsc2]\n\t" \
     "v_fmac_f32 v18, v2, %[bsc2]\n\t" \
@@ -2002,7 +2024,13 @@
     "v_fmac_f32 %[aX12], v6, v22\n\t" \
     "v_fmac_f32 %[aX22], v6, v26\n\t" \
     "s_branch .Lkjoin_%=\n\t" \
+    ".Lr2_%=:\n\t" \
+    "s_waitcnt vmcnt(0)\n\t" \
+    "ds_write_b128 %[rw0], %[st0] offset:18720\n\t" \
+    "s_mov_b64 %[sv], exec\n\ts_and_b64 exec, exec, %[c1]\n\tds_write_b128 %[rw1], %[st1] offset:18720\n\ts_mov_b64 exec, %[sv]\n\t" \
+    "s_waitcnt lgkmcnt(2)\n\t" \
+    "s_branch .Lrj_%=\n\t" \
     ".Lexit_%=:\n\t" \
     : [D0] "+{v[16:31]}"(D0), [aA0] "+v"(accA[0]), [aA1] "+v"(accA[1]), [aA2] "+v"(accA[2]), [aA3] "+v"(accA[3]), [aV00] "+v"(accV[0][0]), [aX00] "+v"(accX[0][0]), [aV01] "+v"(accV[0][1]), [aX01] "+v"(accX[0][1]), [aV02] "+v"(accV[0][2]), [aX02] "+v"(accX[0][2]), [aV10] "+v"(accV[1][0]), [aX10] "+v"(accX[1][0]), [aV11] "+v"(accV[1][1]), [aX11] "+v"(accX[1][1]), [aV12] "+v"(accV[1][2]), [aX12] "+v"(accX[1][2]), [aV20] "+v"(accV[2][0]), [aX20] "+v"(accX[2][0]), [aV21] "+v"(accV[2][1]), [aX21] "+v"(accX[2][1]), [aV22] "+v"(accV[2][2]), [aX22] "+v"(accX[2][2]), [aV30] "+v"(accV[3][0]), [aX30] "+v"(accX[3][0]), [aV31] "+v"(accV[3][1]), [aX31] "+v"(accX[3][1]), [aV32] "+v"(accV[3][2]), [aX32] "+v"(accX[3][2]), [t0] "=&s"(t0_), [t1] "=&s"(t1_), [t2] "=&s"(t2_), [sel] "=&s"(sel_), [pk0] "=&s"(pk0_), [pk1] "=&s"(pk1_), [pk2] "=&s"(pk2_), [sv] "=&s"(sv_) \
-    : [f0] "{v[48:51]}"(f0), [st0] "v"(st0), [st1] "v"(st1), [ringb] "v"(ringb_u), [rw0] "v"(ringw0_u), [rw1] "v"(ringw1_u), [fpa] "v"(fpa_u), [fra] "v"(fra_u), [bsc2] "v"(bsc2), [oscv] "v"(oscv), [s0] "v"(s0), [vx] "v"(vx), [vy] "v"(vy), [vz] "v"(vz), [sm1] "v"(seg.m1), [sm2] "v"(seg.m2), [sm4] "v"(seg.m4), [sm8] "v"(seg.m8), [sm16] "v"(seg.m16), [vrow] "v"(vrow), [hh4] "v"(hh4_u), [hh12] "v"(hh12_u), [w0] "s"(w0), [chan4] "s"(chan4_), [tail] "s"(tail_mask), [sumbase] "s"(sumbase) \
+    : [f0] "{v[48:51]}"(f0), [st0] "v"(st0), [st1] "v"(st1), [ringb] "v"(ringb_u), [rw0] "v"(ringw0_u), [rw1] "v"(ringw1_u), [fpa] "v"(fpa_u), [fra] "v"(fra_u), [bsc2] "v"(bsc2), [oscv] "v"(oscv), [s0] "v"(s0), [vx] "v"(vx), [vy] "v"(vy), [vz] "v"(vz), [sm1] "v"(seg.m1), [sm2] "v"(seg.m2), [sm4] "v"(seg.m4), [sm8] "v"(seg.m8), [sm16] "v"(seg.m16), [vrow] "v"(vrow), [hh4] "v"(hh4_u), [hh12] "v"(hh12_u), [w0] "s"(w0), [chan4] "s"(chan4_), [tail] "s"(tail_mask), [sumbase] "s"(sumbase), [c1] "s"(c1_mask) \
     : "v0", "v1", "v2", "v3", "v4", "v5", "v6", "v7", "v8", "v9", "v10", "v11", "v12", "v13", "v14", "v15", "v52", "v53", "memory", "scc")
```

After: 49.73 (median of 6 runs). +1.9%, better.
